# omron-sinicx/neural-astar

Hardware: AMD Instinct MI355X
Metric: map-instances/s (forward A*) 32x32 Moore-8 @batch 4096 (higher is better)
Workload: dtype f32

## Files before the change

### neural-astar_amd/csrc/nastar_forward_compact_body.inc

```
    extern __shared__ __attribute__((aligned(16))) unsigned char smem[];
    if constexpr (kTicket && kRanked) {
        if (ticket_word != nullptr && blockIdx.x == 0 && threadIdx.x == 0)
            __hip_atomic_store(ticket_word, ticket_value, __ATOMIC_RELAXED, __HIP_MEMORY_SCOPE_SYSTEM);
    }
    const int b = kRanked ? ranked_map(levels, a.B) : placed_map(a.order, a.order_bad, a.B);
    if constexpr (kTicket && !kRanked) {
        if (ticket_word != nullptr && blockIdx.x == 0 && threadIdx.x == 0)
            __hip_atomic_store(ticket_word, ticket_value, __ATOMIC_RELAXED, __HIP_MEMORY_SCOPE_SYSTEM);
        asm volatile("s_nop 0\n s_nop 0\n s_nop 0\n s_nop 0\n s_nop 0\n s_nop 0\n s_nop 0\n s_nop 0\n s_nop 0\n s_nop 0\n s_nop 0\n s_nop 0\n s_nop 0\n s_nop 0");
    }
    if ((unsigned)b >= (unsigned)a.B) return;
    const bool lockstep = !kAsm && (a.flags & NASTAR_FLAG_LOCKSTEP);
    if (lockstep && a.marks != nullptr && a.marks[b] == 0) return;
    const int lane = threadIdx.x;
    CompactDims d = a.d;
    if constexpr (LOGH > 0 && LOGW > 0) {
        d.H = 1 << LOGH;
        d.W = 1 << LOGW;
        d.HW = 1 << (LOGH + LOGW);
        d.nchunks = d.HW >> CCL;
        d.HWp = d.HW;
        d.CPL = (d.nchunks + 63) / 64;
        d.NCp = d.CPL * 64;
        d.magicW = (uint32_t)((1ull << 32) >> LOGW) + 1u;
    }
    CompactLds l;
    if constexpr (kAsm) {
        l = carve_compact_asm_lds(smem, d);
        compact_store_guard_rows(l, d, lane);
    } else l = carve_compact_lds(smem, d);
    const size_t off = (size_t)b * (size_t)d.HW;

    int start_idx, goal_idx;
    constexpr int kLoadIter = (kVec4 && LOGH > 0 && LOGW > 0 && LOGH + LOGW >= 8) ? (1 << (LOGH + LOGW - 8)) : 0;
    bool any_signed = true;
    bool all_unit = false;
    compact_load_map<kVec4, kLoadIter>(d, l, a.cost + off, a.start + off, a.goal + off, a.passable + off, lane, start_idx, goal_idx,
                                       kAsm ? &any_signed : nullptr, kAsm ? &all_unit : nullptr);
#ifdef NASTAR_DEV
    const bool raw = kAsm && !any_signed && !(a.flags & NASTAR_FLAG_ASM_V2) && d.gr >= 0.f && d.omg >= 0.f;
#else
    const bool raw = kAsm && !any_signed && d.gr >= 0.f && d.omg >= 0.f;
#endif
    float* hhv = nullptr;
    bool bad_h0 = false;
    if constexpr (kHeur) {
        hhv = reinterpret_cast<float*>(l.pdir + d.HWp);
        bad_h0 = compact_load_heuristic<kVec4>(d, l, hhv, h0 + off, lane);
    }
    const int gi = goal_idx < 0 ? 0 : goal_idx;
    const int goal_r = (int)row_magic((uint32_t)gi, d.magicW, d.W);
    const int goal_c = gi - goal_r * d.W;

    const CompactLane lc = make_compact_lane<kMasked>(d, lane, nmask);
    int status = NASTAR_OK;
    int iters = 0;
    bool solved = false, coupled = false;
    bool goal_hit = false;
    bool stored_h = false;
    const bool probe = lockstep && a.bitmap != nullptr;
    const int budget = (lockstep && a.t_end != nullptr) ? __builtin_amdgcn_readfirstlane(*a.t_end + 1) : a.max_iters;
    uint32_t bits = 0u;
    uint32_t* const bm = probe ? a.bitmap + (size_t)b * (size_t)a.bitmap_words : nullptr;
    if (kHeur && bad_h0) {
        status = NASTAR_ERR_BAD_HEURISTIC;
    } else if (start_idx < 0 || goal_idx < 0) {
        status = NASTAR_ERR_UNSOLVABLE;
    } else {
#ifdef NASTAR_DEV
        const bool asm4 = raw && !(a.flags & NASTAR_FLAG_ASM_V3);
        const bool no_dive = (a.flags & NASTAR_FLAG_NO_DIVE) != 0;
#else
        const bool asm4 = raw;
#endif
        const bool half = asm4 && d.gr == 0.5f && d.omg == 0.5f;
        if constexpr (kMulti) compact_open_sources<kVec4, kFastDiv, kHeur>(d, l, hhv, a.start + off, lane, goal_r, goal_c, rcp_sqrtW);
        else
        if constexpr (kHeur) {
            if (lane == 0) {
                l.gc[start_idx].x = 0.0f;
                l.cmin[start_idx >> CCL] = cmin_entry(compact_key<kFastDiv>(d, 0.0f, hhv[start_idx], rcp_sqrtW), (uint32_t)start_idx);
                l.pdir[start_idx] = (uint8_t)(PARENT_UNSET | P_PASS);
            }
            wave_sync();
        } else
        compact_open_start<kFastDiv>(d, l, lane, start_idx, goal_r, goal_c, rcp_sqrtW, raw, half);
        int s = 0;
        if constexpr (kAsm) {
#ifdef NASTAR_DEV
            stored_h = asm4 && !no_dive && all_unit && a.cost == a.passable;
#else
            stored_h = asm4 && all_unit && a.cost == a.passable;
#endif
            if (stored_h) {
                const bool start_blocked = l.gc[start_idx].y == 0.0f;
                compact_store_heuristic<LOGW>(l, lane, goal_r, goal_c);
                if (start_blocked && lane == 0) l.gc[start_idx].x = -1.0f;
                wave_sync();
            }
            static_assert(LOGW > 0 && LOGW == LOGH && (CPL_T == 1 || CPL_T == 4) && kFastDiv, "asm loop: 16x16, 32x32, 64x64");
            int* const log_row = kLog ? a.sel_log + (size_t)b * (size_t)a.max_iters : nullptr;
            __builtin_amdgcn_s_setprio(3);
            constexpr bool kD = CPL_T == 4;
#ifdef NASTAR_DEV
            if (asm4 && kD && no_dive) {
                if (half) s = search_loop_asm4<LOGW, kLog, false, true, false>(d.gr, d.omg, d.sqrtW, lane, goal_idx, goal_r, goal_c, a.max_iters, iters, rcp_sqrtW, log_row);
                else s = search_loop_asm4<LOGW, kLog, false, false, false>(d.gr, d.omg, d.sqrtW, lane, goal_idx, goal_r, goal_c, a.max_iters, iters, rcp_sqrtW, log_row);
            } else if (raw && !asm4 && kD && no_dive) {
                s = compact_search_loop_asm3<LOGW, kLog, false>(d, lane, goal_idx, goal_r, goal_c, a.max_iters, iters, rcp_sqrtW, log_row);
            } else if (raw && !asm4) {
                s = compact_search_loop_asm3<LOGW, kLog>(d, lane, goal_idx, goal_r, goal_c, a.max_iters, iters, rcp_sqrtW, log_row);
            } else
#endif
            if (stored_h) {
                s = half ? search_loop_asm5<LOGW, kLog, kD, true>(d.gr, d.omg, d.sqrtW, lane, goal_idx, a.max_iters, iters, rcp_sqrtW, log_row)
                         : search_loop_asm5<LOGW, kLog, kD, false>(d.gr, d.omg, d.sqrtW, lane, goal_idx, a.max_iters, iters, rcp_sqrtW, log_row);
            } else if (asm4) {
                s = half ? search_loop_asm4<LOGW, kLog, kD, true, false>(d.gr, d.omg, d.sqrtW, lane, goal_idx, goal_r, goal_c, a.max_iters, iters, rcp_sqrtW, log_row)
                         : search_loop_asm4<LOGW, kLog, kD, false, false>(d.gr, d.omg, d.sqrtW, lane, goal_idx, goal_r, goal_c, a.max_iters, iters, rcp_sqrtW, log_row);
            } else {
                s = compact_search_loop_asm<LOGW, kLog>(d, lane, goal_idx, goal_r, goal_c, a.max_iters, iters, rcp_sqrtW, log_row);
            }
            __builtin_amdgcn_s_setprio(0);
        } else
        while (iters < budget) {
            uint2 mine;
            s = compact_select<CPL_T>(d, l, lane, mine);
            if (s < 0 || (s == goal_idx && !lockstep)) break;
            if constexpr (kLog) {
                if (lane == 0) a.sel_log[(size_t)b * (size_t)a.max_iters + iters] = s;
            }
            if (probe) {
                if (s == goal_idx) bits |= 1u << (iters & 31);
                if ((iters & 31) == 31) {
                    if (lane == 0) bm[iters >> 5] = bits;
                    bits = 0u;
                }
            }
            ++iters;
            goal_hit |= s == goal_idx;
            if constexpr (kHeur) compact_expand<LOGW, kFastDiv, CPL_T, true>(d, l, lc, lane, s, goal_r, goal_c, rcp_sqrtW, mine, s == goal_idx, hhv);
            else
            compact_expand<LOGW, kFastDiv, CPL_T>(d, l, lc, lane, s, goal_r, goal_c, rcp_sqrtW, mine, s == goal_idx);
        }
        if (probe) {
            if (lane == 0) {
                if (iters & 31) bm[iters >> 5] = bits;
                for (int w = (iters + 31) >> 5; w < a.bitmap_words; ++w) bm[w] = 0u;
            }
            return;
        }
        if (lockstep && goal_hit && lane == 0) l.gc[goal_idx].x = NASTAR_NEG_INF;
        if (kAsm ? (s != -2) : (iters < budget)) {
            if (s < 0) {
                status = NASTAR_ERR_UNSOLVABLE;
            } else {
                if constexpr (kLog) {
                    if (lane == 0) a.sel_log[(size_t)b * (size_t)a.max_iters + iters] = s;
                }
                ++iters;
                solved = true;
                if (a.summary != nullptr || a.marks_out != nullptr) {
                    const int nr = goal_r + lc.dr, nc = goal_c + lc.dc;
                    const bool inb = lc.is_nb & ((unsigned)nr < (unsigned)d.H) & ((unsigned)nc < (unsigned)d.W);
                    const int n = inb ? s + lc.off : s;
                    float2 gg = l.gc[s], gn = l.gc[n];
                    if constexpr (kAsm) {
                        if (stored_h) {
                            gn.y = 1.0f;
                            gg.y = 1.0f;
                            if (s == start_idx) gg = make_float2(0.0f, a.cost[off + s]);
                        }
                    }
                    const float g2 = gg.x + gg.y;
                    uint32_t kn, kg;
                    if constexpr (kHeur) {
                        kn = compact_key<kFastDiv>(d, g2, hhv[n], rcp_sqrtW);
                        kg = compact_key<kFastDiv>(d, gg.x, hhv[s], rcp_sqrtW);
                    } else {
                    kn = compact_key<kFastDiv>(d, g2, d.omg * (heuristic0_fast(nr, nc, goal_r, goal_c) + gn.y), rcp_sqrtW);
                    kg = compact_key<kFastDiv>(d, gg.x, d.omg * (heuristic0_fast(goal_r, goal_c, goal_r, goal_c) + gg.y), rcp_sqrtW);
                    }
                    const bool beats = inb & (gn.x > g2) & ((kn < kg) | ((kn == kg) & (n < s)));
                    coupled = __ballot(beats) != 0ull;
                    if (coupled && a.summary != nullptr && lane == 0) a.summary[NASTAR_SUMMARY_COUPLED] = 1;
                    wave_order();
                }
                if (lane == 0) l.gc[s].x = NASTAR_NEG_INF;
            }
        }
    }
    wave_sync();
    compact_store_hist<kVec4>(d, l, lane, a.hist + off);
    if (probe) return;
    if (lane == 0) {
        a.iters[b] = iters;
        a.status[b] = status;
        if (a.marks_out != nullptr) a.marks_out[b] = coupled ? 1 : 0;
        if (status != NASTAR_OK && a.summary) a.summary[status] = 1;
        if (a.order_out) note_completion(a.order_out, a.B, b);
        if (a.done_counter) note_done(a.done_counter, a.summary, a.B, status != NASTAR_OK || coupled);
    }
    if (goal_idx >= 0 && !(kHeur && bad_h0)) compact_backtrack<(LOGW == LOGH ? LOGW : 0)>(d, l, lane, kMulti ? -1 : start_idx, goal_idx, solved ? d.HW : iters - 1);
    compact_store_outputs<kVec4, false>(d, l, lane, a.hist + off, a.paths + off,
                                        a.packed ? a.packed + (size_t)b * (size_t)(d.HW >> 2) : nullptr);
    const RouteOut ro = kernel_route_args<offsetof(FwdCArgs, route)>();
    if (ro.routes != nullptr) {
        const float start_cost = (kAsm && stored_h) ? a.cost[off + start_idx] : 0.f;
        const int n = route_walk(l.pdir, lane, kMulti ? -1 : start_idx, goal_idx, solved ? d.HW : iters - 1, goal_idx >= 0 && !(kHeur && bad_h0),
                                 [&](int c, uint32_t code) { return compact_parent_of(d, c, code); },
                                 [&](int c) { return (kAsm && stored_h) ? (c == start_idx ? start_cost : 1.0f) : l.gc[c].y; }, ro, b);
        route_fill_tail(ro, b, n, lane);
    }
```

### neural-astar_amd/csrc/nastar_search_asm.hip.h

```cpp
#pragma once
#include "nastar_search_compact.hip.h"

namespace nastar {

template <int LOGW>
struct AsmLayout {
    static constexpr int W = 1 << LOGW;
    static constexpr int HW = W * W;
    static constexpr int CPL = (HW / 16 + 63) / 64;
    static constexpr int GC = W * 8;
    static constexpr int CMIN = GC + HW * 8 + W * 8;
    static constexpr int PDIR = CMIN + CPL * 64 * 8;
    static constexpr int BYTES = PDIR + HW;
};
static_assert(AsmLayout<5>::BYTES == (int)compact_asm_lds_bytes(32, 1024, 64) && AsmLayout<5>::BYTES * 16 == 160 * 1024, "16 maps of 32x32 per CU");
static_assert(AsmLayout<6>::BYTES == (int)compact_asm_lds_bytes(64, 4096, 256) && AsmLayout<4>::BYTES == (int)compact_asm_lds_bytes(16, 256, 64), "host and stream agree");

#define NASTAR_ASM_ENTRY \
        "s_cmp_ge_u32 %[it], %[maxit]\n\t" \
        "s_cbranch_scc1 .Lbudget%=\n\t" \
        "v_mov_b32 v48, -1\n\t" \
        "v_mov_b32 v49, -1\n\t"
 \

#define NASTAR_ASM_READ_1 \
        "ds_read_b64 v[20:21], %[l8] offset:%[CMIN]\n\t"
#define NASTAR_ASM_READ_4 \
        "ds_read_b128 v[12:15], %[l8] offset:%[CMIN]\n\t" \
        "ds_read_b128 v[16:19], %[l8] offset:%[CMIN16]\n\t"
#define NASTAR_ASM_LOOPTOP \
        ".Lloop%=:\n\t" \
        "s_waitcnt lgkmcnt(0)\n\t"
#define NASTAR_ASM_LOCALMIN_1
 \

#define NASTAR_ASM_LOCALMIN_4 \
        "v_min_u32 v21, v13, v15\n\t" \
        "v_min3_u32 v21, v21, v17, v19\n\t" \
        "v_mov_b32 v20, v18\n\t" \
        "v_cmp_eq_u32 vcc, v21, v17\n\t" \
        "v_cmp_eq_u32_e64 s[48:49], v21, v15\n\t" \
        "v_cmp_eq_u32_e64 s[50:51], v21, v13\n\t" \
        "v_cndmask_b32 v20, v20, v16, vcc\n\t" \
        "v_cndmask_b32_e64 v20, v20, v14, s[48:49]\n\t" \
        "v_cndmask_b32_e64 v20, v20, v12, s[50:51]\n\t"
#define NASTAR_ASM_SELECT \
  \
        "v_min_u32_dpp v22, v21, v21 quad_perm:[1,0,3,2] row_mask:0xf bank_mask:0xf\n\t" \
        "s_nop 1\n\t" \
        "v_min_u32_dpp v22, v22, v22 quad_perm:[2,3,0,1] row_mask:0xf bank_mask:0xf\n\t" \
        "s_nop 1\n\t" \
        "v_min_u32_dpp v22, v22, v22 row_half_mirror row_mask:0xf bank_mask:0xf\n\t" \
        "s_nop 1\n\t" \
        "v_min_u32_dpp v22, v22, v22 row_mirror row_mask:0xf bank_mask:0xf\n\t" \
        "s_nop 1\n\t" \
        "v_min_u32_dpp v22, v22, v22 row_bcast:15 row_mask:0xa bank_mask:0xf\n\t" \
        "s_nop 1\n\t" \
        "v_min_u32_dpp v22, v22, v22 row_bcast:31 row_mask:0xc bank_mask:0xf\n\t" \
        "s_nop 0\n\t" \
        "v_readlane_b32 s40, v22, 63\n\t"  \
        "s_cmp_eq_u32 s40, -1\n\t" \
        "s_cbranch_scc1 .Lempty%=\n\t"  \
        "v_cmp_eq_u32 vcc, s40, v21\n\t" \
        "s_ff1_i32_b64 s41, vcc\n\t"  \
        "v_readlane_b32 s42, v20, s41\n\t"  \
        "s_cmp_eq_u32 s42, %[goal]\n\t" \
        "s_cbranch_scc1 .Lgoal%=\n\t"
#define NASTAR_ASM_LOG \
        "s_lshl_b32 s53, %[it], 2\n\t"                     \
        "v_mov_b32 v53, s53\n\t"                                                                                           \
        "v_mov_b32 v54, s42\n\t"                                                                                           \
        "s_mov_b64 exec, 1\n\t"                                                                                            \
        "global_store_dword v53, v54, %[logp]\n\t"                                                                         \
        "s_mov_b64 exec, -1\n\t"
#define NASTAR_ASM_EXPAND \
        "s_add_u32 %[it], %[it], 1\n\t" \
  \
        "s_lshr_b32 s43, s42, %[LOGW]\n\t"  \
        "s_and_b32 s44, s42, %[WM1]\n\t"  \
        "s_and_b32 s45, s42, 0xfffffff0\n\t"  \
        "v_add_u32 v23, s43, %[dr]\n\t" \
        "v_add_u32 v24, s44, %[dc]\n\t" \
        "v_max_u32 v23, v23, v24\n\t" \
        "v_cmp_gt_u32 vcc, %[W], v23\n\t"  \
        "v_mov_b32 v24, s42\n\t" \
        "v_mov_b32 v46, s45\n\t" \
        "v_cndmask_b32_e64 v46, v24, v46, %[mchk]\n\t"  \
        "v_add_u32 v46, v46, %[off]\n\t" \
        "s_and_b64 s[54:55], vcc, %[mnb]\n\t"  \
        "v_cndmask_b32 v46, v24, v46, vcc\n\t"  \
        "v_lshlrev_b32 v27, 3, v24\n\t" \
        "v_lshlrev_b32 v26, 3, v46\n\t" \
        "ds_read_b64 v[28:29], v27 offset:%[GC]\n\t"  \
        "ds_read_b64 v[30:31], v26 offset:%[GC]\n\t"  \
  \
        "v_lshrrev_b32 v32, %[LOGW], v46\n\t" \
        "v_and_b32 v33, %[WM1], v46\n\t" \
        "v_subrev_u32 v32, %[gr], v32\n\t" \
        "v_subrev_u32 v33, %[gc], v33\n\t" \
        "v_cvt_f32_i32 v32, v32\n\t" \
        "v_cvt_f32_i32 v33, v33\n\t" \
        "v_mul_f32 v34, v32, v32\n\t" \
        "v_mul_f32 v35, v33, v33\n\t" \
        "v_add_f32 v34, v34, v35\n\t" \
        "v_sqrt_f32 v34, v34\n\t" \
        "v_add_f32_e64 v35, |v32|, |v33|\n\t" \
        "v_min_f32_e64 v32, |v32|, |v33|\n\t" \
        "v_sub_f32 v35, v35, v32\n\t"  \
        "v_mul_f32 v34, 0x3a83126f, v34\n\t"  \
        "v_add_f32 v34, v35, v34\n\t"  \
        "s_lshr_b32 s47, s42, 4\n\t" \
        "s_lshl_b32 s47, s47, 3\n\t"  \
        "s_and_b32 s46, s42, 15\n\t" \
        "s_add_u32 s46, s46, 16\n\t"  \
        "s_waitcnt lgkmcnt(0)\n\t" \
        "v_add_f32 v34, v34, v31\n\t"  \
        "v_mul_f32 v34, %[comg], v34\n\t"  \
        "v_add_f32 v40, v28, v29\n\t"  \
        "v_cndmask_b32_e64 v41, v30, v40, %[mnb]\n\t"  \
        "v_mul_f32 v41, %[cgr], v41\n\t" \
        "v_add_f32 v41, v41, v34\n\t"  \
        "v_mul_f32 v42, %[crcp], v41\n\t"  \
        "v_fma_f32 v43, -v42, %[csq], v41\n\t" \
        "v_fma_f32 v42, v43, %[crcp], v42\n\t" \
        "v_ashrrev_i32 v43, 31, v42\n\t" \
        "v_cmp_eq_u32 vcc, s46, %[lane]\n\t" \
        "v_bitop3_b32 v47, v43, v42, %[msb] bitop3:0x36\n\t"  \
        "v_cndmask_b32_e64 v45, %[vinf], v40, s[54:55]\n\t"  \
        "v_cndmask_b32 v44, %[loc], %[vinf], vcc\n\t"  \
        "v_lshrrev_b32 v50, 4, v46\n\t" \
        "v_lshlrev_b32 v50, 3, v50\n\t"  \
        "v_mov_b32 v52, s47\n\t" \
  \
        "s_mov_b64 exec, 0x100\n\t" \
        "ds_write_b32 v27, %[vminf] offset:%[GC]\n\t" \
        "ds_write_b64 v52, v[48:49] offset:%[CMIN]\n\t" \
        "s_mov_b64 exec, -1\n\t" \
        "v_cmpx_gt_f32 vcc, v30, v44\n\t"  \
        "v_cmpx_ge_f32 vcc, 0x7f7fffff, v30\n\t"  \
        "ds_min_u64 v50, v[46:47] offset:%[CMIN]\n\t" \
        "s_mov_b64 exec, -1\n\t" \
        "v_cmpx_gt_f32 vcc, v30, v45\n\t"  \
        "ds_write_b32 v26, v40 offset:%[GC]\n\t"  \
        "ds_write_b8 v46, %[pcode] offset:%[PDIR]\n\t"  \
        "ds_min_u64 v50, v[46:47] offset:%[CMIN]\n\t"  \
        "s_mov_b64 exec, -1\n\t"
#define NASTAR_ASM_LOOPEND \
        "s_cmp_lt_u32 %[it], %[maxit]\n\t" \
        "s_cbranch_scc1 .Lloop%=\n" \
        ".Lbudget%=:\n\t" \
        "s_waitcnt lgkmcnt(0)\n\t"  \
        "s_mov_b32 %[sel], -2\n\t" \
        "s_branch .Lend%=\n" \
        ".Lempty%=:\n\t" \
        "s_mov_b32 %[sel], -1\n\t" \
        "s_branch .Lend%=\n" \
        ".Lgoal%=:\n\t" \
        "s_mov_b32 %[sel], s42\n" \
        ".Lend%=:\n\t"
#define NASTAR_ASM_OPERANDS \
        : [it] "+s"(it), [sel] "=s"(sel) \
        : [l8] "v"(v_l8), [lane] "v"(lane), [dr] "v"(v_dr), [dc] "v"(v_dc), [off] "v"(v_off), [pcode] "v"(v_pcode), \
          [vinf] "v"(v_inf), [vminf] "v"(v_minf), [loc] "v"(v_loc), [goal] "s"(goal_idx), [gr] "s"(goal_r), [gc] "s"(goal_c), \
          [maxit] "s"(max_iters), [cgr] "s"(d.gr), [comg] "s"(d.omg), [csq] "s"(d.sqrtW), [crcp] "s"(rcp_sqrtW), \
          [mnb] "s"(m_nb), [mchk] "s"(m_chk), [msb] "s"(msb), [logp] "s"(logp), \
          [GC] "i"(L::GC), [CMIN] "i"(L::CMIN), [CMIN16] "i"(L::CMIN + 16), [PDIR] "i"(L::PDIR), [LOGW] "i"(LOGW), [WM1] "i"(L::W - 1), [W] "i"(L::W) \
        : "memory", "vcc", "scc", "v20", "v21", "v22", "v23", "v24", "v26", "v27", "v28", "v29", "v30", "v31", "v32", "v33", \
          "v34", "v35", "v40", "v41", "v42", "v43", "v44", "v45", "v46", "v47", "v48", "v49", "v50", "v52", "s40", "s41", "s42", \
          "s43", "s44", "s45", "s46", "s47", "s50", "s51", "s52", "s54", "s55", "s53", "v53", "v54", "v12", "v13", "v14", "v15", "v16", "v17", "v18", "v19", "s48", "s49"

template <int LOGW, bool kLog>
__device__ __forceinline__ int compact_search_loop_asm(const CompactDims& d, int lane, int goal_idx, int goal_r, int goal_c,
                                                       int max_iters, int& iters, float rcp_sqrtW, int* log_row)
{
    using L = AsmLayout<LOGW>;
    static_assert((L::CPL == 1 || L::CPL == 4) && L::HW >= 256, "1 or 4 chunk minima per lane, chunks inside one map row");
    int dr, dc;
    neighbour_delta(lane & 7, dr, dc);
    const bool is_nb = lane < 8, is_chk = (lane & 48) == 16;
    const int v_dr = is_nb ? dr : 0, v_dc = is_nb ? dc : 0;
    const int v_off = is_nb ? dr * L::W + dc : (is_chk ? (lane & 15) : 0);
    const uint32_t v_pcode = P_PASS | (uint32_t)(lane & 7);
    const uint32_t v_l8 = (uint32_t)lane * 8u * L::CPL;
    const float v_inf = NASTAR_POS_INF, v_minf = NASTAR_NEG_INF;
    const float v_loc = is_chk ? NASTAR_NEG_INF : NASTAR_POS_INF;
    const unsigned long long m_nb = 0xFFull, m_chk = 0xFFFF0000ull;
    const uint32_t msb = 0x80000000u;
    int it = __builtin_amdgcn_readfirstlane(iters);
    goal_idx = __builtin_amdgcn_readfirstlane(goal_idx);
    goal_r = __builtin_amdgcn_readfirstlane(goal_r);
    goal_c = __builtin_amdgcn_readfirstlane(goal_c);
    max_iters = __builtin_amdgcn_readfirstlane(max_iters);
    int sel;
    unsigned long long logp = reinterpret_cast<unsigned long long>(log_row);
#define NASTAR_ASM_BODY(N, LOGPART) \
    NASTAR_ASM_ENTRY NASTAR_ASM_READ_##N NASTAR_ASM_LOOPTOP NASTAR_ASM_LOCALMIN_##N NASTAR_ASM_SELECT LOGPART NASTAR_ASM_EXPAND \
        NASTAR_ASM_READ_##N NASTAR_ASM_LOOPEND
    if constexpr (L::CPL == 1) {
        if constexpr (kLog) asm volatile(NASTAR_ASM_BODY(1, NASTAR_ASM_LOG) NASTAR_ASM_OPERANDS);
        else asm volatile(NASTAR_ASM_BODY(1, ) NASTAR_ASM_OPERANDS);
    } else {
        if constexpr (kLog) asm volatile(NASTAR_ASM_BODY(4, NASTAR_ASM_LOG) NASTAR_ASM_OPERANDS);
        else asm volatile(NASTAR_ASM_BODY(4, ) NASTAR_ASM_OPERANDS);
    }
#undef NASTAR_ASM_BODY
    iters = it;
    return sel;
}

}
```

### neural-astar_amd/csrc/nastar_search_asm3.hip.h

```cpp
#pragma once
#include "nastar_search_asm.hip.h"

namespace nastar {

#define NASTAR_ASM3_SELECT \
  \
        "v_min_u32_dpp v22, v21, v21 quad_perm:[1,0,3,2] row_mask:0xf bank_mask:0xf\n\t" \
        "v_min_u32_dpp v23, v21, v21 quad_perm:[2,3,0,1] row_mask:0xf bank_mask:0xf\n\t" \
        "v_min_u32_dpp v22, v21, v22 quad_perm:[3,2,1,0] row_mask:0xf bank_mask:0xf\n\t" \
        "v_min_u32 v22, v22, v23\n\t" \
        "s_add_u32 %[it], %[it], 1\n\t" \
        "s_nop 0\n\t" \
        "v_min_u32_dpp v22, v22, v22 row_half_mirror row_mask:0xf bank_mask:0xf\n\t" \
        "s_nop 1\n\t" \
        "v_min_u32_dpp v22, v22, v22 row_mirror row_mask:0xf bank_mask:0xf\n\t" \
        "s_nop 1\n\t" \
        "v_min_u32_dpp v22, v22, v22 row_bcast:15 row_mask:0xa bank_mask:0xf\n\t" \
        "s_nop 1\n\t" \
        "v_min_u32_dpp v22, v22, v22 row_bcast:31 row_mask:0xc bank_mask:0xf\n\t" \
        "s_nop 0\n\t" \
        "v_readlane_b32 s40, v22, 63\n\t"  \
        "s_cmp_eq_u32 s40, -1\n\t" \
        "s_cbranch_scc1 .Lempty%=\n\t"  \
        "v_cmp_eq_u32 vcc, s40, v21\n\t" \
        "s_ff1_i32_b64 s41, vcc\n\t"  \
        "v_readlane_b32 s42, v20, s41\n\t"  \
        "s_cmp_eq_u32 s42, %[goal]\n\t" \
        "s_cbranch_scc1 .Lgoal%=\n\t"
#define NASTAR_ASM3_LOG \
        "s_lshl_b32 s53, %[it], 2\n\t"                     \
        "s_sub_u32 s53, s53, 4\n\t"                                                                                        \
        "v_mov_b32 v53, s53\n\t"                                                                                           \
        "v_mov_b32 v54, s42\n\t"                                                                                           \
        "s_mov_b64 exec, 1\n\t"                                                                                            \
        "global_store_dword v53, v54, %[logp]\n\t"                                                                         \
        "s_mov_b64 exec, -1\n\t"
#define NASTAR_ASM3_LOOPEND \
        "s_cmp_lt_u32 %[it], %[maxit]\n\t" \
        "s_cbranch_scc1 .Lloop%=\n" \
        ".Lbudget%=:\n\t" \
        "s_waitcnt lgkmcnt(0)\n\t"  \
        "s_mov_b32 %[sel], -2\n\t" \
        "s_branch .Lend%=\n" \
        ".Lempty%=:\n\t" \
        "s_sub_u32 %[it], %[it], 1\n\t"  \
        "s_mov_b32 %[sel], -1\n\t" \
        "s_branch .Lend%=\n" \
        ".Lgoal%=:\n\t" \
        "s_sub_u32 %[it], %[it], 1\n\t"  \
        "s_mov_b32 %[sel], s42\n" \
        ".Lend%=:\n\t"

#define NASTAR_ASM3_X_PREFIX \
        "s_lshr_b32 s43, s42, %[LOGW]\n\t"  \
        "s_and_b32 s44, s42, %[WM1]\n\t"  \
        "v_add_u32 v32, s43, %[dr]\n\t"  \
        "v_and_b32 v33, s44, %[cmask]\n\t"  \
        "v_add_u32 v33, v33, %[dcc]\n\t"  \
        "v_mov_b32 v24, s42\n\t" \
        "v_max_u32 v23, v32, v33\n\t" \
        "v_lshl_add_u32 v46, v32, %[LOGW], v33\n\t"  \
        "v_cmp_gt_u32 vcc, %[W], v23\n\t"  \
        "v_lshlrev_b32 v27, 3, v24\n\t" \
        "ds_read_b64 v[28:29], v27 offset:%[GC]\n\t"  \
        "s_and_b64 s[54:55], vcc, %[mnb]\n\t"  \
        "v_cndmask_b32 v46, v24, v46, vcc\n\t"  \
        "v_lshlrev_b32 v26, 3, v46\n\t" \
        "v_lshrrev_b32 v50, 4, v46\n\t" \
        "v_lshlrev_b32 v50, 3, v50\n\t"
#define NASTAR_ASM3_X_CLOSE \
  \
        "s_mov_b64 exec, 0x100\n\t" \
        "ds_write_b32 v27, %[vminf] offset:%[GC]\n\t" \
        "ds_write_b64 v50, v[48:49] offset:%[CMIN]\n\t" \
        "s_mov_b64 exec, -1\n\t"
#define NASTAR_ASM3_X_READCELL \
        "ds_read_b64 v[30:31], v26 offset:%[GC]\n\t"
#define NASTAR_ASM3_X_HEUR \
  \
        "v_sad_u32 v35, v32, %[gr], 0\n\t"  \
        "v_sad_u32 v36, v33, %[gc], 0\n\t"  \
        "v_max_u32 v37, v35, v36\n\t"  \
        "v_mul_u32_u24 v34, v35, v35\n\t" \
        "v_mad_u32_u24 v34, v36, v36, v34\n\t" \
        "v_cvt_f32_u32 v34, v34\n\t" \
        "v_sqrt_f32 v34, v34\n\t" \
        "v_cvt_f32_u32 v37, v37\n\t"  \
        "v_mul_f32 v34, 0x3a83126f, v34\n\t"  \
        "v_add_f32 v34, v37, v34\n\t"
#define NASTAR_ASM3_X_WAIT \
        "s_waitcnt lgkmcnt(0)\n\t"
#define NASTAR_ASM3_X_KEY \
        "v_add_f32 v34, v34, v31\n\t"  \
        "v_add_f32 v40, v28, v29\n\t"  \
        "v_mul_f32 v34, %[comg], v34\n\t"  \
        "v_cndmask_b32_e64 v41, v30, v40, %[mnb]\n\t"  \
        "v_mul_f32 v41, %[cgr], v41\n\t" \
        "v_add_f32 v41, v41, v34\n\t"  \
        "v_mul_f32 v42, %[crcp], v41\n\t"  \
        "v_fma_f32 v43, -v42, %[csq], v41\n\t" \
        "v_fma_f32 v47, v43, %[crcp], v42\n\t"
#define NASTAR_ASM3_X_RELAX(SET55) \
  \
        "v_cmp_class_f32_e64 s[58:59], v30, %[cls]\n\t"  \
        "s_mov_b64 exec, s[54:55]\n\t" \
        "v_cmpx_gt_f32 vcc, v30, v40\n\t"  \
        SET55 \
        "ds_write_b32 v26, v40 offset:%[GC]\n\t"  \
        "ds_write_b8 v46, %[pcode] offset:%[PDIR]\n\t"  \
        "s_or_b64 exec, exec, s[58:59]\n\t" \
        "ds_min_u64 v50, v[46:47] offset:%[CMIN]\n\t"  \
        "s_mov_b64 exec, -1\n\t"
#define NASTAR_ASM3_EXPAND_(INIT55, SET55) \
    NASTAR_ASM3_X_PREFIX NASTAR_ASM3_X_CLOSE NASTAR_ASM3_X_READCELL INIT55 NASTAR_ASM3_X_HEUR NASTAR_ASM3_X_WAIT NASTAR_ASM3_X_KEY \
        NASTAR_ASM3_X_RELAX(SET55)
#define NASTAR_ASM3_EXPAND NASTAR_ASM3_EXPAND_(, )
#define NASTAR_ASM3_EXPAND_DIVE NASTAR_ASM3_EXPAND_(, "v_cmp_lt_u32_e64 s[60:61], v47, s40\n\t")

#define NASTAR_ASM3_DIVE_TEST \
        "s_cmp_ge_u32 %[it], %[maxit]\n\t" \
        "s_cbranch_scc1 .Lbudget%=\n\t" \
        "s_cmp_lg_u64 s[60:61], 0\n\t"  \
        "s_cbranch_scc1 .Ldive%=\n\t"
#define NASTAR_ASM3_DIVE_LOOKUP \
        ".Ldive%=:\n\t" \
        "v_cndmask_b32_e64 v55, v48, v47, s[60:61]\n\t"  \
        "s_nop 1\n\t" \
        "v_min_u32_dpp v56, v55, v55 quad_perm:[1,0,3,2] row_mask:0xf bank_mask:0xf\n\t" \
        "v_min_u32_dpp v57, v55, v55 quad_perm:[2,3,0,1] row_mask:0xf bank_mask:0xf\n\t" \
        "v_min_u32_dpp v56, v55, v56 quad_perm:[3,2,1,0] row_mask:0xf bank_mask:0xf\n\t" \
        "v_min_u32 v56, v56, v57\n\t" \
        "s_add_u32 %[it], %[it], 1\n\t" \
        "s_nop 0\n\t" \
        "v_min_u32_dpp v56, v56, v56 row_half_mirror row_mask:0xf bank_mask:0xf\n\t" \
        "s_nop 0\n\t" \
        "v_readfirstlane_b32 s56, v56\n\t"  \
        "s_mov_b32 s40, s56\n\t"  \
        "s_nop 0\n\t" \
        "v_cmp_eq_u32 vcc, s56, v55\n\t" \
        "s_ff1_i32_b64 s41, vcc\n\t"  \
        "v_readlane_b32 s42, v46, s41\n\t"  \
        "s_cmp_eq_u32 s42, %[goal]\n\t" \
        "s_cbranch_scc1 .Lgoal%=\n" \
        ".Lselected%=:\n\t"
#define NASTAR_ASM3_EXITS \
        ".Lbudget%=:\n\t" \
        "s_waitcnt lgkmcnt(0)\n\t"  \
        "s_mov_b32 %[sel], -2\n\t" \
        "s_branch .Lend%=\n" \
        ".Lempty%=:\n\t" \
        "s_sub_u32 %[it], %[it], 1\n\t" \
        "s_mov_b32 %[sel], -1\n\t" \
        "s_branch .Lend%=\n" \
        ".Lgoal%=:\n\t" \
        "s_sub_u32 %[it], %[it], 1\n\t" \
        "s_mov_b32 %[sel], s42\n" \
        ".Lend%=:\n\t"


#define NASTAR_ASM3_OPERANDS \
        : [it] "+s"(it), [sel] "=s"(sel) \
        : [l8] "v"(v_l8), [dr] "v"(v_dr), [cmask] "v"(v_cmask), [dcc] "v"(v_dcc), [pcode] "v"(v_pcode), [cls] "v"(v_cls), \
          [vminf] "v"(v_minf), [goal] "s"(goal_idx), [gr] "s"(goal_r), [gc] "s"(goal_c), \
          [maxit] "s"(max_iters), [cgr] "s"(d.gr), [comg] "s"(d.omg), [csq] "s"(d.sqrtW), [crcp] "s"(rcp_sqrtW), \
          [mnb] "s"(m_nb), [logp] "s"(logp), \
          [GC] "i"(L::GC), [CMIN] "i"(L::CMIN), [CMIN16] "i"(L::CMIN + 16), [PDIR] "i"(L::PDIR), [LOGW] "i"(LOGW), [WM1] "i"(L::W - 1), [W] "i"(L::W) \
        : "memory", "vcc", "scc", "v20", "v21", "v22", "v23", "v24", "v26", "v27", "v28", "v29", "v30", "v31", "v32", "v33", \
          "v34", "v35", "v36", "v37", "v40", "v41", "v42", "v43", "v46", "v47", "v48", "v49", "v50", "s40", "s41", "s42", \
          "s43", "s44", "s54", "s55", "s53", "v53", "v54", "v12", "v13", "v14", "v15", "v16", "v17", "v18", "v19", "s48", "s49", \
          "s50", "s51", "v55", "v56", "v57", "s56", "s58", "s59", "s60", "s61"

template <int LOGW, bool kLog, bool kDive = true>
__device__ __forceinline__ int compact_search_loop_asm3(const CompactDims& d, int lane, int goal_idx, int goal_r, int goal_c,
                                                        int max_iters, int& iters, float rcp_sqrtW, int* log_row)
{
    using L = AsmLayout<LOGW>;
    static_assert((L::CPL == 1 || L::CPL == 4) && L::HW >= 256, "1 or 4 chunk minima per lane, chunks inside one map row");
    int dr, dc;
    neighbour_delta(lane & 7, dr, dc);
    const bool is_nb = lane < 8, is_chk = (lane & 48) == 16;
    const int v_dr = is_nb ? dr : 0;
    const int v_dcc = is_nb ? dc : (is_chk ? (lane & 15) : 0);
    const uint32_t v_cmask = is_chk ? 0xFFFFFFF0u : 0xFFFFFFFFu;
    const uint32_t v_cls = is_chk ? 0x1F8u : 0u;
    const uint32_t v_pcode = P_PASS | (uint32_t)(lane & 7);
    const uint32_t v_l8 = (uint32_t)lane * 8u * L::CPL;
    const float v_minf = NASTAR_NEG_INF;
    const unsigned long long m_nb = 0xFFull;
    int it = __builtin_amdgcn_readfirstlane(iters);
    goal_idx = __builtin_amdgcn_readfirstlane(goal_idx);
    goal_r = __builtin_amdgcn_readfirstlane(goal_r);
    goal_c = __builtin_amdgcn_readfirstlane(goal_c);
    max_iters = __builtin_amdgcn_readfirstlane(max_iters);
    int sel;
    unsigned long long logp = reinterpret_cast<unsigned long long>(log_row);
#define NASTAR_ASM3_BODY(N, LOGPART) \
    NASTAR_ASM_ENTRY NASTAR_ASM_READ_##N NASTAR_ASM_LOOPTOP NASTAR_ASM_LOCALMIN_##N NASTAR_ASM3_SELECT LOGPART NASTAR_ASM3_EXPAND \
        NASTAR_ASM_READ_##N NASTAR_ASM3_LOOPEND
#define NASTAR_ASM3_BODY_DIVE(N, LOGPART) \
    NASTAR_ASM_ENTRY NASTAR_ASM_READ_##N "s_branch .Lsel%=\n" NASTAR_ASM3_DIVE_LOOKUP LOGPART NASTAR_ASM3_EXPAND_DIVE NASTAR_ASM_READ_##N \
        NASTAR_ASM3_DIVE_TEST ".Lsel%=:\n\t" "s_waitcnt lgkmcnt(0)\n\t" NASTAR_ASM_LOCALMIN_##N NASTAR_ASM3_SELECT \
        "s_branch .Lselected%=\n" NASTAR_ASM3_EXITS
    if constexpr (L::CPL == 1) {
        if constexpr (kLog) asm volatile(NASTAR_ASM3_BODY(1, NASTAR_ASM3_LOG) NASTAR_ASM3_OPERANDS);
        else asm volatile(NASTAR_ASM3_BODY(1, ) NASTAR_ASM3_OPERANDS);
    } else if constexpr (kDive) {
        if constexpr (kLog) asm volatile(NASTAR_ASM3_BODY_DIVE(4, NASTAR_ASM3_LOG) NASTAR_ASM3_OPERANDS);
        else asm volatile(NASTAR_ASM3_BODY_DIVE(4, ) NASTAR_ASM3_OPERANDS);
    } else {
        if constexpr (kLog) asm volatile(NASTAR_ASM3_BODY(4, NASTAR_ASM3_LOG) NASTAR_ASM3_OPERANDS);
        else asm volatile(NASTAR_ASM3_BODY(4, ) NASTAR_ASM3_OPERANDS);
    }
#undef NASTAR_ASM3_BODY_DIVE
#undef NASTAR_ASM3_BODY
    iters = it;
    return sel;
}

}
```

### neural-astar_amd/csrc/nastar_search_asm4.hip.h

```cpp
#pragma once
#include "nastar_search_asm3.hip.h"

namespace nastar {

template <int LOGW>
struct AsmLayoutUnit {
    static constexpr int W = 1 << LOGW;
    static constexpr int HW = W * W;
    static constexpr int CPL = (HW / 16 + 63) / 64;
    static constexpr int GC = 0;
    static constexpr int CMIN = HW * 4;
    static constexpr int PDIR = CMIN + CPL * 64 * 8;
    static constexpr int BYTES = PDIR + HW;
};

#define NASTAR_ASM4_ENTRY \
        "s_cmp_ge_u32 %[it], %[maxit]\n\t" \
        "s_cbranch_scc1 .Lbudget%=\n\t" \
        "v_mov_b32 v48, %[goal]\n\t"  \
        "v_mov_b32 v49, -1\n\t"

#define NASTAR_ASM4_SELECT \
        "v_min_u32_dpp v22, v21, v21 quad_perm:[1,0,3,2] row_mask:0xf bank_mask:0xf\n\t" \
        "v_min_u32_dpp v23, v21, v21 quad_perm:[2,3,0,1] row_mask:0xf bank_mask:0xf\n\t" \
        "v_min_u32_dpp v22, v21, v22 quad_perm:[3,2,1,0] row_mask:0xf bank_mask:0xf\n\t" \
        "v_min_u32 v22, v22, v23\n\t" \
        "s_nop 1\n\t" \
        "v_min_u32_dpp v22, v22, v22 row_half_mirror row_mask:0xf bank_mask:0xf\n\t" \
        "s_nop 1\n\t" \
        "v_min_u32_dpp v22, v22, v22 row_mirror row_mask:0xf bank_mask:0xf\n\t" \
        "s_nop 1\n\t" \
        "v_min_u32_dpp v22, v22, v22 row_bcast:15 row_mask:0xa bank_mask:0xf\n\t" \
        "s_nop 1\n\t" \
        "v_min_u32_dpp v22, v22, v22 row_bcast:31 row_mask:0xc bank_mask:0xf\n\t" \
        "s_nop 0\n\t" \
        "v_readlane_b32 s40, v22, 63\n\t"  \
        "s_add_u32 %[it], %[it], 1\n\t"  \
        "s_nop 0\n\t" \
        "v_cmp_eq_u32 vcc, s40, v21\n\t" \
        "s_ff1_i32_b64 s41, vcc\n\t" \
        "v_readlane_b32 s42, v20, s41\n\t" \
        "s_cmp_eq_u32 s42, %[goal]\n\t" \
        "s_cbranch_scc1 .Lgoal%=\n\t"

#define NASTAR_ASM4_X_PREFIX(SH, RDS) \
        "s_lshr_b32 s43, s42, %[LOGW]\n\t"  \
        "s_and_b32 s44, s42, %[WM1]\n\t"  \
        "v_add_u32 v32, s43, %[dr]\n\t"  \
        "v_and_b32 v33, s44, %[cmask]\n\t" \
        "v_add_u32 v33, v33, %[dcc]\n\t"  \
        "v_mov_b32 v24, s42\n\t" \
        "v_max_u32 v23, v32, v33\n\t" \
        "v_lshl_add_u32 v46, v32, %[LOGW], v33\n\t"  \
        "v_cmp_gt_u32 vcc, %[W], v23\n\t"  \
        "v_lshlrev_b32 v27, " SH ", v24\n\t" \
        RDS  \
        "v_lshlrev_b32 v26, " SH ", v46\n\t" \
        "s_and_b64 s[54:55], vcc, %[mnb]\n\t"  \
        "v_lshrrev_b32 v50, 4, v46\n\t" \
        "v_lshlrev_b32 v50, 3, v50\n\t"

#define NASTAR_ASM4_X_KEY(ADDH, ADDG, MULH, MULG) \
        ADDH  \
        ADDG  \
        MULH  \
        "v_cndmask_b32_e64 v41, v30, v40, %[mnb]\n\t"  \
        MULG  \
        "v_add_f32 v41, v41, v34\n\t"  \
        "v_mul_f32 v42, %[crcp], v41\n\t"  \
        "v_fma_f32 v43, -v42, %[csq], v41\n\t" \
        "v_fma_f32 v47, v43, %[crcp], v42\n\t"

#define NASTAR_ASM4_DIVE_LOOKUP \
        ".Ldive%=:\n\t" \
        "v_cndmask_b32_e64 v55, v49, v47, s[60:61]\n\t" \
        "s_nop 1\n\t" \
        "v_min_u32_dpp v56, v55, v55 quad_perm:[1,0,3,2] row_mask:0xf bank_mask:0xf\n\t" \
        "v_min_u32_dpp v57, v55, v55 quad_perm:[2,3,0,1] row_mask:0xf bank_mask:0xf\n\t" \
        "v_min_u32_dpp v56, v55, v56 quad_perm:[3,2,1,0] row_mask:0xf bank_mask:0xf\n\t" \
        "v_min_u32 v56, v56, v57\n\t" \
        "s_add_u32 %[it], %[it], 1\n\t" \
        "s_nop 0\n\t" \
        "v_min_u32_dpp v56, v56, v56 row_half_mirror row_mask:0xf bank_mask:0xf\n\t" \
        "s_nop 0\n\t" \
        "v_readfirstlane_b32 s56, v56\n\t" \
        "s_mov_b32 s40, s56\n\t" \
        "s_nop 0\n\t" \
        "v_cmp_eq_u32 vcc, s56, v55\n\t" \
        "s_ff1_i32_b64 s41, vcc\n\t" \
        "v_readlane_b32 s42, v46, s41\n\t" \
        "s_cmp_eq_u32 s42, %[goal]\n\t" \
        "s_cbranch_scc1 .Lgoal%=\n" \
        ".Lselected%=:\n\t"

#define NASTAR_ASM4_EXITS \
        ".Lbudget%=:\n\t" \
        "s_waitcnt lgkmcnt(0)\n\t"  \
        "s_mov_b32 %[sel], -2\n\t" \
        "s_branch .Lend%=\n" \
        ".Lgoal%=:\n\t" \
        "s_sub_u32 %[it], %[it], 1\n\t"  \
        "s_mov_b32 %[sel], s42\n\t" \
        "s_mov_b32 %[mkey], s40\n" \
        ".Lend%=:\n\t"
#define NASTAR_ASM4_LOOPEND \
        "s_cmp_lt_u32 %[it], %[maxit]\n\t" \
        "s_cbranch_scc1 .Lloop%=\n" \
        NASTAR_ASM4_EXITS

#define NASTAR_ASM4_OPERANDS \
        : [it] "+s"(it), [sel] "=s"(sel), [mkey] "=s"(mkey) \
        : [l8] "v"(v_l8), [dr] "v"(v_dr), [cmask] "v"(v_cmask), [dcc] "v"(v_dcc), [pcode] "v"(v_pcode), [cls] "v"(v_cls), \
          [vminf] "v"(v_minf), [goal] "s"(goal_idx), [gr] "s"(goal_r), [gc] "s"(goal_c), \
          [maxit] "s"(max_iters), [cgr] "s"(cgr), [comg] "s"(comg), [csq] "s"(csq), [crcp] "s"(rcp_sqrtW), \
          [mnb] "s"(m_nb), [logp] "s"(logp), \
          [GC] "i"(GC), [CMIN] "i"(CMIN), [CMIN16] "i"(CMIN + 16), [PDIR] "i"(PDIR), [LOGW] "i"(LOGW), [WM1] "i"((1 << LOGW) - 1), [W] "i"(1 << LOGW) \
        : "memory", "vcc", "scc", "v20", "v21", "v22", "v23", "v24", "v26", "v27", "v28", "v29", "v30", "v31", "v32", "v33", \
          "v34", "v35", "v36", "v37", "v40", "v41", "v42", "v43", "v46", "v47", "v48", "v49", "v50", "s40", "s41", "s42", \
          "s43", "s44", "s54", "s55", "s53", "v53", "v54", "v12", "v13", "v14", "v15", "v16", "v17", "v18", "v19", "s48", "s49", \
          "s50", "s51", "v55", "v56", "v57", "s56", "s58", "s59", "s60", "s61"

template <int LOGW, bool kLog, bool kDive, bool kHalf, bool kUnit>
__device__ __forceinline__ int search_loop_asm4(float cgr, float comg, float csq, int lane, int goal_idx, int goal_r, int goal_c,
                                                int max_iters, int& iters, float rcp_sqrtW, int* log_row)
{
    using LG = AsmLayout<LOGW>;
    using LU = AsmLayoutUnit<LOGW>;
    constexpr int CPL = LG::CPL;
    constexpr int GC = kUnit ? LU::GC : LG::GC;
    constexpr int CMIN = kUnit ? LU::CMIN : LG::CMIN;
    constexpr int PDIR = kUnit ? LU::PDIR : LG::PDIR;
    static_assert((CPL == 1 || CPL == 4) && LG::HW >= 256, "1 or 4 chunk minima per lane, chunks inside one map row");
    int dr, dc;
    neighbour_delta(lane & 7, dr, dc);
    const bool is_nb = lane < 8, is_chk = (lane & 48) == 16;
    const int v_dr = is_nb ? dr : 0;
    const int v_dcc = is_nb ? dc : (is_chk ? (lane & 15) : 0);
    const uint32_t v_cmask = is_chk ? 0xFFFFFFF0u : 0xFFFFFFFFu;
    const uint32_t v_cls = is_chk ? 0x1F8u : 0u;
    const uint32_t v_pcode = P_PASS | (uint32_t)(lane & 7);
    const uint32_t v_l8 = (uint32_t)lane * 8u * CPL;
    const float v_minf = NASTAR_NEG_INF;
    const unsigned long long m_nb = 0xFFull;
    int it = __builtin_amdgcn_readfirstlane(iters);
    goal_idx = __builtin_amdgcn_readfirstlane(goal_idx);
    goal_r = __builtin_amdgcn_readfirstlane(goal_r);
    goal_c = __builtin_amdgcn_readfirstlane(goal_c);
    max_iters = __builtin_amdgcn_readfirstlane(max_iters);
    int sel;
    uint32_t mkey = 0;
    unsigned long long logp = reinterpret_cast<unsigned long long>(log_row);
#define NASTAR_A4_SH_G "3"
#define NASTAR_A4_SH_U "2"
#define NASTAR_A4_RDS_G "ds_read_b64 v[28:29], v27 offset:%[GC]\n\t"
#define NASTAR_A4_RDS_U "ds_read_b32 v28, v27 offset:%[GC]\n\t"
#define NASTAR_A4_RDC_G "ds_read_b64 v[30:31], v26 offset:%[GC]\n\t"
#define NASTAR_A4_RDC_U "ds_read_b32 v30, v26 offset:%[GC]\n\t"
#define NASTAR_A4_ADDH_G "v_add_f32 v34, v34, v31\n\t"
#define NASTAR_A4_ADDH_U "v_add_f32 v34, 1.0, v34\n\t"
#define NASTAR_A4_ADDG_G "v_add_f32 v40, v28, v29\n\t"
#define NASTAR_A4_ADDG_U "v_add_f32 v40, 1.0, v28\n\t"
#define NASTAR_A4_MULH "v_mul_f32 v34, %[comg], v34\n\t"
#define NASTAR_A4_MULG "v_mul_f32 v41, %[cgr], v41\n\t"
#define NASTAR_A4_EXPAND(L, MH, MG, SET55) \
    NASTAR_ASM4_X_PREFIX(NASTAR_A4_SH_##L, NASTAR_A4_RDS_##L) NASTAR_ASM3_X_CLOSE NASTAR_A4_RDC_##L NASTAR_ASM3_X_HEUR NASTAR_ASM3_X_WAIT \
        NASTAR_ASM4_X_KEY(NASTAR_A4_ADDH_##L, NASTAR_A4_ADDG_##L, MH, MG) NASTAR_ASM3_X_RELAX(SET55)
#define NASTAR_A4_BODY(N, L, MH, MG, LOGPART) \
    NASTAR_ASM4_ENTRY NASTAR_ASM_READ_##N NASTAR_ASM_LOOPTOP NASTAR_ASM_LOCALMIN_##N NASTAR_ASM4_SELECT LOGPART NASTAR_A4_EXPAND(L, MH, MG, ) \
        NASTAR_ASM_READ_##N NASTAR_ASM4_LOOPEND
#define NASTAR_A4_BODY_DIVE(N, L, MH, MG, LOGPART) \
    NASTAR_ASM4_ENTRY NASTAR_ASM_READ_##N "s_branch .Lsel%=\n" NASTAR_ASM4_DIVE_LOOKUP LOGPART \
        NASTAR_A4_EXPAND(L, MH, MG, "v_cmp_lt_u32_e64 s[60:61], v47, s40\n\t") NASTAR_ASM_READ_##N NASTAR_ASM3_DIVE_TEST ".Lsel%=:\n\t" \
        "s_waitcnt lgkmcnt(0)\n\t" NASTAR_ASM_LOCALMIN_##N NASTAR_ASM4_SELECT "s_branch .Lselected%=\n" NASTAR_ASM4_EXITS
#define NASTAR_A4_RUN2(BODY, N, L, MH, MG) \
    do { \
        if constexpr (kLog) asm volatile(BODY(N, L, MH, MG, NASTAR_ASM3_LOG) NASTAR_ASM4_OPERANDS); \
        else asm volatile(BODY(N, L, MH, MG, ) NASTAR_ASM4_OPERANDS); \
    } while (0)
#define NASTAR_A4_RUN(BODY, N) \
    do { \
        if constexpr (kUnit && kHalf) NASTAR_A4_RUN2(BODY, N, U, , ); \
        else if constexpr (kUnit) NASTAR_A4_RUN2(BODY, N, U, NASTAR_A4_MULH, NASTAR_A4_MULG); \
        else if constexpr (kHalf) NASTAR_A4_RUN2(BODY, N, G, , ); \
        else NASTAR_A4_RUN2(BODY, N, G, NASTAR_A4_MULH, NASTAR_A4_MULG); \
    } while (0)
    if constexpr (CPL == 1 && kDive) NASTAR_A4_RUN(NASTAR_A4_BODY_DIVE, 1);
    else if constexpr (CPL == 1) NASTAR_A4_RUN(NASTAR_A4_BODY, 1);
    else if constexpr (kDive) NASTAR_A4_RUN(NASTAR_A4_BODY_DIVE, 4);
    else NASTAR_A4_RUN(NASTAR_A4_BODY, 4);
#undef NASTAR_A4_RUN
#undef NASTAR_A4_RUN2
#undef NASTAR_A4_BODY_DIVE
#undef NASTAR_A4_BODY
#undef NASTAR_A4_EXPAND
    iters = it;
    return (sel >= 0 && mkey == 0xFFFFFFFFu) ? -1 : sel;
}


}
```

### neural-astar_amd/csrc/nastar_search_asm5.hip.h

```cpp
#pragma once
#include "nastar_search_asm4.hip.h"

namespace nastar {

#define NASTAR_ASM5_ENTRY \
        "s_mov_b32 s55, 0\n\t"
#define NASTAR_ASM5_X_PREFIX \
        "v_and_b32 v46, s42, %[cmask]\n\t"  \
        "v_lshlrev_b32_e64 v27, 3, s42\n\t" \
        "v_add_u32 v46, v46, %[delta]\n\t"  \
        "ds_read_b32 v28, v27 offset:%[GC]\n\t"  \
        "v_lshlrev_b32 v26, 3, v46\n\t"
#define NASTAR_ASM5_X_CLOSE \
  \
        "s_mov_b64 exec, 0x100\n\t" \
        "ds_write_b32 v27, %[vminf] offset:%[GC]\n\t" \
        "s_mov_b64 exec, -1\n\t"
#define NASTAR_ASM5_X_READCELL \
        "ds_read_b64 v[30:31], v26 offset:%[GC]\n\t"
#define NASTAR_ASM5_X_SHADOW \
  \
        "v_readlane_b32 s54, %[colmask], s42\n\t" \
        "v_lshrrev_b32 v50, 4, v46\n\t" \
        "v_lshlrev_b32 v50, 3, v50\n\t"  \
        "s_mov_b64 exec, 0x100\n\t" \
        "ds_write_b64 v50, v[48:49] offset:%[CMIN]\n\t" \
        "s_mov_b64 exec, -1\n\t"
#define NASTAR_ASM5_X_WAIT \
        "s_waitcnt lgkmcnt(1)\n\t"
#define NASTAR_ASM5_X_KEY(MULH, MULG) \
        "v_add_f32 v40, 1.0, v28\n\t"  \
        MULH  \
        "v_cndmask_b32_e64 v41, v30, v40, %[mnb]\n\t"  \
        MULG  \
        "v_add_f32 v41, v41, v31\n\t"  \
        "v_mul_f32 v42, %[crcp], v41\n\t"  \
        "v_fma_f32 v43, -v42, %[csq], v41\n\t" \
        "v_fma_f32 v47, v43, %[crcp], v42\n\t"
#define NASTAR_ASM5_MULH "v_mul_f32 v31, %[comg], v31\n\t"
#define NASTAR_ASM5_MULG "v_mul_f32 v41, %[cgr], v41\n\t"

#define NASTAR_ASM5_OPERANDS \
        : [it] "+s"(it), [sel] "=s"(sel), [mkey] "=s"(mkey) \
        : [l8] "v"(v_l8), [cmask] "v"(v_cmask), [colmask] "v"(v_colmask), [delta] "v"(v_delta), [pcode] "v"(v_pcode), \
          [cls] "v"(v_cls), [vminf] "v"(v_minf), [goal] "s"(goal_idx), \
          [maxit] "s"(max_iters), [cgr] "s"(cgr), [comg] "s"(comg), [csq] "s"(csq), [crcp] "s"(rcp_sqrtW), \
          [mnb] "s"(m_nb), [logp] "s"(logp), \
          [GC] "i"(GC), [CMIN] "i"(CMIN), [CMIN16] "i"(CMIN + 16), [PDIR] "i"(PDIR) \
        : "memory", "vcc", "scc", "v20", "v21", "v22", "v23", "v26", "v27", "v28", "v30", "v31", \
          "v40", "v41", "v42", "v43", "v46", "v47", "v48", "v49", "v50", "s40", "s41", "s42", \
          "s54", "s55", "s53", "v53", "v54", "v12", "v13", "v14", "v15", "v16", "v17", "v18", "v19", "s48", "s49", \
          "s50", "s51", "v55", "v56", "v57", "s56", "s58", "s59", "s60", "s61"

template <int LOGW, bool kLog, bool kDive, bool kHalf>
__device__ __forceinline__ int search_loop_asm5(float cgr, float comg, float csq, int lane, int goal_idx, int max_iters, int& iters,
                                                float rcp_sqrtW, int* log_row)
{
    using LG = AsmLayout<LOGW>;
    constexpr int CPL = LG::CPL;
    constexpr int GC = LG::GC;
    constexpr int CMIN = LG::CMIN;
    constexpr int PDIR = LG::PDIR;
    static_assert((CPL == 1 || CPL == 4) && LG::HW >= 256, "1 or 4 chunk minima per lane, chunks inside one map row");
    int dr, dc;
    neighbour_delta(lane & 7, dr, dc);
    const bool is_nb = lane < 8, is_chk = (lane & 48) == 16;
    const int v_delta = is_nb ? dr * (1 << LOGW) + dc : (is_chk ? (lane & 15) : 0);
    const uint32_t v_cmask = is_chk ? 0xFFFFFFF0u : 0xFFFFFFFFu;
    const uint32_t v_cls = is_chk ? 0x1F8u : 0u;
    const uint32_t v_pcode = P_PASS | (uint32_t)(lane & 7);
    const uint32_t v_l8 = (uint32_t)lane * 8u * CPL;
    const float v_minf = NASTAR_NEG_INF;
    const unsigned long long m_nb = 0xFFull;
    const int col = lane & ((1 << LOGW) - 1);
    const uint32_t v_colmask = 0xFFu & ~(col == 0 ? 0x29u : 0u) & ~(col == (1 << LOGW) - 1 ? 0x94u : 0u);
    int it = __builtin_amdgcn_readfirstlane(iters);
    goal_idx = __builtin_amdgcn_readfirstlane(goal_idx);
    max_iters = __builtin_amdgcn_readfirstlane(max_iters);
    int sel;
    uint32_t mkey = 0;
    unsigned long long logp = reinterpret_cast<unsigned long long>(log_row);
#define NASTAR_A5_EXPAND(MH, MG, SET55) \
    NASTAR_ASM5_X_PREFIX NASTAR_ASM5_X_CLOSE NASTAR_ASM5_X_READCELL NASTAR_ASM5_X_SHADOW NASTAR_ASM5_X_WAIT NASTAR_ASM5_X_KEY(MH, MG) \
        NASTAR_ASM3_X_RELAX(SET55)
#define NASTAR_A5_BODY(N, MH, MG, LOGPART) \
    NASTAR_ASM5_ENTRY NASTAR_ASM4_ENTRY NASTAR_ASM_READ_##N NASTAR_ASM_LOOPTOP NASTAR_ASM_LOCALMIN_##N NASTAR_ASM4_SELECT LOGPART NASTAR_A5_EXPAND(MH, MG, ) \
        NASTAR_ASM_READ_##N NASTAR_ASM4_LOOPEND
#define NASTAR_A5_BODY_DIVE(N, MH, MG, LOGPART) \
    NASTAR_ASM5_ENTRY NASTAR_ASM4_ENTRY NASTAR_ASM_READ_##N "s_branch .Lsel%=\n" NASTAR_ASM4_DIVE_LOOKUP LOGPART \
        NASTAR_A5_EXPAND(MH, MG, "v_cmp_lt_u32_e64 s[60:61], v47, s40\n\t") NASTAR_ASM_READ_##N NASTAR_ASM3_DIVE_TEST ".Lsel%=:\n\t" \
        "s_waitcnt lgkmcnt(0)\n\t" NASTAR_ASM_LOCALMIN_##N NASTAR_ASM4_SELECT "s_branch .Lselected%=\n" NASTAR_ASM4_EXITS
#define NASTAR_A5_RUN2(BODY, N, MH, MG) \
    do { \
        if constexpr (kLog) asm volatile(BODY(N, MH, MG, NASTAR_ASM3_LOG) NASTAR_ASM5_OPERANDS); \
        else asm volatile(BODY(N, MH, MG, ) NASTAR_ASM5_OPERANDS); \
    } while (0)
#define NASTAR_A5_RUN(BODY, N) \
    do { \
        if constexpr (kHalf) NASTAR_A5_RUN2(BODY, N, , ); \
        else NASTAR_A5_RUN2(BODY, N, NASTAR_ASM5_MULH, NASTAR_ASM5_MULG); \
    } while (0)
    if constexpr (CPL == 1 && kDive) NASTAR_A5_RUN(NASTAR_A5_BODY_DIVE, 1);
    else if constexpr (CPL == 1) NASTAR_A5_RUN(NASTAR_A5_BODY, 1);
    else if constexpr (kDive) NASTAR_A5_RUN(NASTAR_A5_BODY_DIVE, 4);
    else NASTAR_A5_RUN(NASTAR_A5_BODY, 4);
#undef NASTAR_A5_RUN
#undef NASTAR_A5_RUN2
#undef NASTAR_A5_BODY_DIVE
#undef NASTAR_A5_BODY
#undef NASTAR_A5_EXPAND
    iters = it;
    return (sel >= 0 && mkey == 0xFFFFFFFFu) ? -1 : sel;
}

template <int LOGW>
__device__ __forceinline__ void compact_store_heuristic(const CompactLds& l, int lane, int goal_r, int goal_c)
{
    constexpr int W = 1 << LOGW, HW = W * W;
    static_assert(W <= 64 && HW % 64 == 0, "a lane's cells share one column");
    const int c = lane & (W - 1);
    const int dcol = c > goal_c ? c - goal_c : goal_c - c;
    const uint32_t dc2 = (uint32_t)(dcol * dcol);
#pragma unroll 4
    for (int k = 0; k < HW / 64; ++k) {
        const int i = lane + 64 * k;
        const int r = i >> LOGW;
        const int drow = r > goal_r ? r - goal_r : goal_r - r;
        const uint32_t cheb = (uint32_t)(drow > dcol ? drow : dcol);
        const float euc = __builtin_amdgcn_sqrtf((float)((uint32_t)(drow * drow) + dc2));
        const float h0 = (float)cheb + 0.001f * euc;
        l.gc[i].y = h0 + 1.0f;
    }
}

}
```

### neural-astar_amd/csrc/nastar_search_compact.hip.h

```cpp
#pragma once
#include "nastar_search.hip.h"

namespace nastar {

constexpr int CCL = 4;
constexpr int CCSZ = 1 << CCL;

struct CompactDims {
    int H, W, HW;
    int nchunks;
    int HWp;
    int CPL;
    int NCp;
    uint32_t magicW;
    float gr, omg, sqrtW;
};

struct CompactLds {
    float2* gc;
    unsigned long long* cmin;
    uint8_t* pdir;
    uint32_t* dump;
};

__host__ __device__ inline size_t compact_lds_bytes(int HWp, int NCp) { return (size_t)HWp * 9 + (size_t)NCp * 8 + 256; }

__host__ __device__ constexpr size_t compact_asm_lds_bytes(int W, int HWp, int NCp) { return (size_t)HWp * 9 + (size_t)NCp * 8 + (size_t)W * 16; }
__host__ __device__ inline bool compact_asm_shape(int H, int W) { return H == W && (W == 16 || W == 32 || W == 64); }

__host__ __device__ inline size_t compact_launch_lds_bytes(int H, int W, int HWp, int NCp, bool asm_stream)
{
    return (asm_stream && compact_asm_shape(H, W)) ? compact_asm_lds_bytes(W, HWp, NCp) : compact_lds_bytes(HWp, NCp);
}

__host__ __device__ inline size_t compact_heur_lds_bytes(int HWp, int NCp) { return compact_lds_bytes(HWp, NCp) + (size_t)HWp * 4; }

__device__ __forceinline__ CompactLds carve_compact_lds(unsigned char* smem, const CompactDims& d)
{
    CompactLds l;
    l.gc = reinterpret_cast<float2*>(smem);
    l.cmin = reinterpret_cast<unsigned long long*>(l.gc + d.HWp);
    l.dump = reinterpret_cast<uint32_t*>(l.cmin + d.NCp);
    l.pdir = reinterpret_cast<uint8_t*>(l.dump + 64);
    return l;
}

__device__ __forceinline__ CompactLds carve_compact_asm_lds(unsigned char* smem, const CompactDims& d)
{
    CompactLds l;
    l.gc = reinterpret_cast<float2*>(smem) + d.W;
    l.cmin = reinterpret_cast<unsigned long long*>(l.gc + d.HW + d.W);
    l.pdir = reinterpret_cast<uint8_t*>(l.cmin + d.NCp);
    l.dump = nullptr;
    return l;
}

__device__ __forceinline__ void compact_store_guard_rows(const CompactLds& l, const CompactDims& d, int lane)
{
    for (int i = lane; i < 2 * d.W; i += 64) l.gc[i < d.W ? i - d.W : d.HW + i - d.W] = make_float2(NASTAR_NEG_INF, 0.f);
}

__device__ __forceinline__ unsigned long long cmin_entry(uint32_t key, uint32_t idx)
{
    return ((unsigned long long)key << 32) | (unsigned long long)idx;
}

template <bool kFastDiv>
__device__ __forceinline__ uint32_t compact_key(const CompactDims& d, float G, float hh, float rcp_sqrtW)
{
    const float f = d.gr * G + hh;
    float q;
    if constexpr (kFastDiv) {
        const float q0 = f * rcp_sqrtW;
        const float rem = __builtin_fmaf(-q0, d.sqrtW, f);
        q = __builtin_fmaf(rem, rcp_sqrtW, q0);
    } else {
        q = f / d.sqrtW;
    }
    return f32_to_ord(q);
}

__device__ __forceinline__ float heuristic0_fast(int r, int c, int goal_r, int goal_c)
{
    const float a = (float)(r - goal_r);
    const float b = (float)(c - goal_c);
    const float dr = fabsf(a), dc = fabsf(b);
    const float cheb = (dr + dc) - fminf(dr, dc);
    const float euc = sqrt_rn_int(a * a + b * b);
    return cheb + 0.001f * euc;
}

template <bool kVec4, int ITER = 0>
__device__ __forceinline__ void compact_load_map(const CompactDims& d, const CompactLds& l, const float* __restrict__ cost,
                                                 const float* __restrict__ start, const float* __restrict__ goal,
                                                 const float* __restrict__ passable, int lane, int& start_idx, int& goal_idx,
                                                 bool* any_signed = nullptr, bool* all_unit = nullptr)
{
    int sidx = -1, gidx = -1;
    bool sgn = false, nun = false;
    if constexpr (kVec4) {
        const float4* s4 = reinterpret_cast<const float4*>(start);
        const float4* g4 = reinterpret_cast<const float4*>(goal);
        const float4* c4 = reinterpret_cast<const float4*>(cost);
        const float4* p4 = reinterpret_cast<const float4*>(passable);
        auto place = [&](int q, const float4& sv, const float4& gv, const float4& cv, const float4& pv) {
            const int i = q << 2;
            if (sv.x != 0.f) sidx = i;
            if (sv.y != 0.f) sidx = i + 1;
            if (sv.z != 0.f) sidx = i + 2;
            if (sv.w != 0.f) sidx = i + 3;
            if (gv.x != 0.f) gidx = i;
            if (gv.y != 0.f) gidx = i + 1;
            if (gv.z != 0.f) gidx = i + 2;
            if (gv.w != 0.f) gidx = i + 3;
            sgn |= !(cv.x >= 0.f) | !(cv.y >= 0.f) | !(cv.z >= 0.f) | !(cv.w >= 0.f);
            nun |= ((cv.x != 0.f) & (cv.x != 1.f)) | ((cv.y != 0.f) & (cv.y != 1.f)) | ((cv.z != 0.f) & (cv.z != 1.f)) | ((cv.w != 0.f) & (cv.w != 1.f));
            float4 lo, hi;
            lo.x = pv.x != 0.f ? NASTAR_POS_INF : NASTAR_NEG_INF;
            lo.y = cv.x;
            lo.z = pv.y != 0.f ? NASTAR_POS_INF : NASTAR_NEG_INF;
            lo.w = cv.y;
            hi.x = pv.z != 0.f ? NASTAR_POS_INF : NASTAR_NEG_INF;
            hi.y = cv.z;
            hi.z = pv.w != 0.f ? NASTAR_POS_INF : NASTAR_NEG_INF;
            hi.w = cv.w;
            *reinterpret_cast<float4*>(l.gc + i) = lo;
            *reinterpret_cast<float4*>(l.gc + i + 2) = hi;
            const uint32_t m = (PARENT_UNSET | (pv.x != 0.f ? P_PASS : 0u)) | ((PARENT_UNSET | (pv.y != 0.f ? P_PASS : 0u)) << 8) |
                               ((PARENT_UNSET | (pv.z != 0.f ? P_PASS : 0u)) << 16) |
                               ((PARENT_UNSET | (pv.w != 0.f ? P_PASS : 0u)) << 24);
            *reinterpret_cast<uint32_t*>(l.pdir + i) = m;
        };
        if constexpr (ITER > 0) {
            constexpr int G = ITER < 4 ? ITER : 4;
            static_assert(ITER % G == 0, "groups of up to 4 iterations");
            const bool same_cp = passable == cost;
            for (int base = 0; base < ITER; base += G) {
                float4 sv[G], gv[G], cv[G], pv[G];
#pragma unroll
                for (int k = 0; k < G; ++k) {
                    const int q = lane + (base + k) * 64;
                    sv[k] = s4[q];
                    gv[k] = g4[q];
                    cv[k] = c4[q];
                }
                if (same_cp) {
#pragma unroll
                    for (int k = 0; k < G; ++k) pv[k] = cv[k];
                } else {
#pragma unroll
                    for (int k = 0; k < G; ++k) pv[k] = p4[lane + (base + k) * 64];
                }
#pragma unroll
                for (int k = 0; k < G; ++k) place(lane + (base + k) * 64, sv[k], gv[k], cv[k], pv[k]);
            }
        } else {
            const int n4 = d.HW >> 2;
            for (int q = lane; q < n4; q += 64) place(q, s4[q], g4[q], c4[q], p4[q]);
        }
    } else {
        for (int i = lane; i < d.HW; i += 64) {
            if (start[i] != 0.f) sidx = i;
            if (goal[i] != 0.f) gidx = i;
            const float pv = passable[i];
            sgn |= !(cost[i] >= 0.f);
            nun |= (cost[i] != 0.f) & (cost[i] != 1.f);
            l.gc[i] = make_float2(pv != 0.f ? NASTAR_POS_INF : NASTAR_NEG_INF, cost[i]);
            l.pdir[i] = (uint8_t)(PARENT_UNSET | (pv != 0.f ? P_PASS : 0u));
        }
    }
    for (int i = d.HW + lane; i < d.HWp; i += 64) l.gc[i] = make_float2(NASTAR_NEG_INF, 0.f);
    start_idx = wave_max_i32(sidx);
    goal_idx = wave_max_i32(gidx);
    const unsigned long long idle = cmin_entry(0xFFFFFFFFu, (uint32_t)(goal_idx < 0 ? 0 : goal_idx));
    for (int c = lane; c < d.NCp; c += 64) l.cmin[c] = idle;
    if (any_signed != nullptr) *any_signed = __ballot(sgn) != 0ull;
    if (all_unit != nullptr) *all_unit = __ballot(nun) == 0ull;
    wave_sync();
}

template <bool kVec4>
__device__ __forceinline__ bool compact_load_heuristic(const CompactDims& d, const CompactLds& l, float* hhv, const float* __restrict__ h0, int lane)
{
    bool bad = false;
    if constexpr (kVec4) {
        const float4* h4 = reinterpret_cast<const float4*>(h0);
        const int n4 = d.HW >> 2;
        for (int q = lane; q < n4; q += 64) {
            const float4 hv = h4[q];
            const float4 lo = *reinterpret_cast<const float4*>(l.gc + (q << 2));
            const float4 hi = *reinterpret_cast<const float4*>(l.gc + (q << 2) + 2);
            bad = bad || !(fabsf(hv.x) < NASTAR_POS_INF) || !(fabsf(hv.y) < NASTAR_POS_INF) || !(fabsf(hv.z) < NASTAR_POS_INF) || !(fabsf(hv.w) < NASTAR_POS_INF);
            float4 o;
            o.x = d.omg * (hv.x + lo.y);
            o.y = d.omg * (hv.y + lo.w);
            o.z = d.omg * (hv.z + hi.y);
            o.w = d.omg * (hv.w + hi.w);
            *reinterpret_cast<float4*>(hhv + (q << 2)) = o;
        }
    } else {
        for (int i = lane; i < d.HW; i += 64) {
            const float hv = h0[i];
            bad |= !(fabsf(hv) < NASTAR_POS_INF);
            hhv[i] = d.omg * (hv + l.gc[i].y);
        }
    }
    for (int i = d.HW + lane; i < d.HWp; i += 64) hhv[i] = 0.f;
    const bool any_bad = __ballot(bad) != 0ull;
    wave_sync();
    return any_bad;
}

template <bool kFastDiv>
__device__ __forceinline__ void compact_open_start(const CompactDims& d, const CompactLds& l, int lane, int sidx, int goal_r,
                                                   int goal_c, float rcp_sqrtW, bool raw_key = false, bool half_key = false)
{
    if (lane == 0) {
        const int r = (int)row_magic((uint32_t)sidx, d.magicW, d.W);
        const int c = sidx - r * d.W;
        const float hh = (half_key ? 1.0f : d.omg) * (heuristic0_fast(r, c, goal_r, goal_c) + l.gc[sidx].y);
        uint32_t k0 = compact_key<kFastDiv>(d, 0.0f, hh, rcp_sqrtW);
        if (raw_key) k0 = __float_as_uint(ord_to_f32(k0));
        l.gc[sidx].x = 0.0f;
        l.cmin[sidx >> CCL] = cmin_entry(k0, (uint32_t)sidx);
        l.pdir[sidx] = (uint8_t)(PARENT_UNSET | P_PASS);
    }
    wave_sync();
}

template <bool kVec4, bool kFastDiv, bool kHeur>
__device__ __forceinline__ void compact_open_sources(const CompactDims& d, const CompactLds& l, const float* hhv, const float* __restrict__ start,
                                                     int lane, int goal_r, int goal_c, float rcp_sqrtW)
{
    auto open = [&](int i) {
        float hh;
        if constexpr (kHeur) {
            hh = hhv[i];
        } else {
            const int r = (int)row_magic((uint32_t)i, d.magicW, d.W);
            const int c = i - r * d.W;
            hh = d.omg * (heuristic0_fast(r, c, goal_r, goal_c) + l.gc[i].y);
        }
        const uint32_t k0 = compact_key<kFastDiv>(d, 0.0f, hh, rcp_sqrtW);
        l.gc[i].x = 0.0f;
        l.pdir[i] = (uint8_t)(PARENT_UNSET | P_PASS);
        atomicMin(&l.cmin[i >> CCL], cmin_entry(k0, (uint32_t)i));
    };
    if constexpr (kVec4) {
        const float4* s4 = reinterpret_cast<const float4*>(start);
        const int n4 = d.HW >> 2;
        for (int q = lane; q < n4; q += 64) {
            const float4 sv = s4[q];
            if (sv.x != 0.f) open(q << 2);
            if (sv.y != 0.f) open((q << 2) + 1);
            if (sv.z != 0.f) open((q << 2) + 2);
            if (sv.w != 0.f) open((q << 2) + 3);
        }
    } else {
        for (int i = lane; i < d.HW; i += 64)
            if (start[i] != 0.f) open(i);
    }
    wave_sync();
}

template <int CPL_T>
__device__ __forceinline__ int compact_select(const CompactDims& d, const CompactLds& l, int lane, uint2& mine)
{
    uint2 best;
    if constexpr (CPL_T == 1) {
        const unsigned long long e = l.cmin[lane];
        best.x = (uint32_t)e;
        best.y = (uint32_t)(e >> 32);
    } else {
        const int cpl = CPL_T > 0 ? CPL_T : d.CPL;
        const uint2* p = reinterpret_cast<const uint2*>(l.cmin) + lane * cpl;
        best = p[0];
        if constexpr (CPL_T > 0) {
#pragma unroll
            for (int c = 1; c < CPL_T; ++c) {
                const uint2 e = p[c];
                if (e.y < best.y) best = e;
            }
        } else {
            for (int c = 1; c < cpl; ++c) {
                const uint2 e = p[c];
                if (e.y < best.y) best = e;
            }
        }
    }
    mine = best;
    const uint32_t M = wave_min_scalar_u32(best.y);
    const int L = __builtin_ctzll(__ballot(best.y == M));
    const int s = __builtin_amdgcn_readlane((int)best.x, L);
    return M == KEY_INF ? -1 : s;
}

struct CompactLane {
    int dr, dc, off;
    bool is_nb;
    bool is_chk;
    uint32_t pcode;
};

template <bool kMasked = false>
__device__ __forceinline__ CompactLane make_compact_lane(const CompactDims& d, int lane, uint32_t nmask = 0u)
{
    CompactLane lc;
    neighbour_delta(lane & 7, lc.dr, lc.dc);
    lc.is_nb = kMasked ? neighbour_enabled(lane, nmask) : lane < 8;
    lc.is_chk = (lane & 48) == 16;
    lc.off = lc.dr * d.W + lc.dc;
    lc.pcode = P_PASS | (uint32_t)(lane & 7);
    return lc;
}

template <int LOGW, bool kFastDiv, int CPL_T, bool kHeur = false>
__device__ __forceinline__ void compact_expand(const CompactDims& d, const CompactLds& l, const CompactLane& lc, int lane, int s,
                                               int goal_r, int goal_c, float rcp_sqrtW, const uint2 mine, const bool keep_open = false,
                                               const float* hhv = nullptr)
{
    int r, c;
    if constexpr (LOGW) {
        r = s >> LOGW;
        c = s & ((1 << LOGW) - 1);
    } else {
        r = (int)row_magic((uint32_t)s, d.magicW, d.W);
        c = s - r * d.W;
    }
    const int cbase = s & ~(CCSZ - 1);
    const int nr = r + lc.dr, nc = c + lc.dc;
    const bool inb = lc.is_nb & ((unsigned)nr < (unsigned)d.H) & ((unsigned)nc < (unsigned)d.W);
    const int il = inb ? s + lc.off : (lc.is_chk ? cbase + (lane & (CCSZ - 1)) : s);
    const float2 gs = l.gc[s];
    const float2 gl = l.gc[il];
    float hh;
    if constexpr (kHeur) {
        hh = hhv[il];
    } else {
    int rl, cl;
    if constexpr (LOGW) {
        rl = il >> LOGW;
        cl = il & ((1 << LOGW) - 1);
    } else {
        rl = (int)row_magic((uint32_t)il, d.magicW, d.W);
        cl = il - rl * d.W;
    }
    const float h0 = heuristic0_fast(rl, cl, goal_r, goal_c);
    hh = d.omg * (h0 + gl.y);
    }
    const float g2 = gs.x + gs.y;
    const bool upd = inb & (gl.x > g2);
    const uint32_t k = compact_key<kFastDiv>(d, lc.is_nb ? g2 : gl.x, hh, rcp_sqrtW);
    const bool open_l = lc.is_chk & (fabsf(gl.x) < NASTAR_POS_INF) & ((il != s) | keep_open);
    const uint32_t kk = open_l ? k : KEY_INF;
    const uint32_t mc = row_min16_u32(kk);
    const unsigned long long firstm = __ballot(lc.is_chk & (kk == mc));
    const uint32_t Mc = (uint32_t)__builtin_amdgcn_readlane((int)mc, 16);
    const uint32_t ci = (uint32_t)(cbase + __builtin_ctzll(firstm) - 16);
    uint32_t* const dmp = l.dump + lane;
    float* const g_dst = upd ? &l.gc[il].x : ((lane == 8 && !keep_open) ? &l.gc[s].x : reinterpret_cast<float*>(dmp));
    uint8_t* const p_dst = upd ? &l.pdir[il] : reinterpret_cast<uint8_t*>(dmp);
    *g_dst = upd ? g2 : NASTAR_NEG_INF;
    *p_dst = (uint8_t)lc.pcode;
    if constexpr (CPL_T == 1) {
        const bool owner = lane == (s >> CCL);
        uint2 e;
        e.x = owner ? ci : mine.x;
        e.y = owner ? Mc : mine.y;
        reinterpret_cast<uint2*>(l.cmin)[lane] = e;
    } else {
        if (lane == 16) l.cmin[s >> CCL] = cmin_entry(Mc, ci);
    }
    atomicMin(upd ? &l.cmin[il >> CCL] : &l.cmin[lane], upd ? cmin_entry(k, (uint32_t)il) : ~0ull);
    wave_order();
}

__device__ __forceinline__ int compact_parent_of(const CompactDims& d, int n, uint32_t code)
{
    int dr, dc;
    neighbour_delta((int)code, dr, dc);
    return n - (dr * d.W + dc);
}

template <int LOGW = 0>
__device__ __forceinline__ void compact_backtrack(const CompactDims& d, const CompactLds& l, int lane, int start_idx, int goal_idx,
                                                  int cap)
{
    if (lane == 0) {
        auto parent_of = [&](int n, uint32_t code) -> int {
            if constexpr (LOGW > 0 && LOGW <= 6) {
                constexpr int W = 1 << LOGW;
                constexpr unsigned long long LUT =
                    ((unsigned long long)(uint8_t)(int8_t)(-W - 1)) | ((unsigned long long)(uint8_t)(int8_t)(-W) << 8) |
                    ((unsigned long long)(uint8_t)(int8_t)(-W + 1) << 16) | ((unsigned long long)(uint8_t)(int8_t)(-1) << 24) |
                    ((unsigned long long)(uint8_t)(int8_t)(1) << 32) | ((unsigned long long)(uint8_t)(int8_t)(W - 1) << 40) |
                    ((unsigned long long)(uint8_t)(int8_t)(W) << 48) | ((unsigned long long)(uint8_t)(int8_t)(W + 1) << 56);
                return n - (int)(int8_t)(LUT >> (code * 8u));
            } else {
                return compact_parent_of(d, n, code);
            }
        };
        uint32_t m = l.pdir[goal_idx];
        l.pdir[goal_idx] = (uint8_t)(m | P_PATH);
        uint32_t code = m & P_DIRMASK;
        if (code != PARENT_UNSET) {
            int loc = parent_of(goal_idx, code);
            for (int k = 0; k < cap; ++k) {
                uint32_t ml = l.pdir[loc];
                l.pdir[loc] = (uint8_t)(ml | P_PATH);
                if (loc == start_idx) break;
                uint32_t cd = ml & P_DIRMASK;
                if (cd == PARENT_UNSET) break;
                loc = parent_of(loc, cd);
            }
        }
    }
    wave_sync();
}

template <bool kVec4>
__device__ __forceinline__ void compact_store_hist(const CompactDims& d, const CompactLds& l, int lane, float* __restrict__ hist)
{
    if constexpr (kVec4) {
        const int n4 = d.HW >> 2;
        float4* h4 = reinterpret_cast<float4*>(hist);
        for (int q = lane; q < n4; q += 64) {
            const uint32_t m = *reinterpret_cast<const uint32_t*>(l.pdir + (q << 2));
            const float4 lo = *reinterpret_cast<const float4*>(l.gc + (q << 2));
            const float4 hi = *reinterpret_cast<const float4*>(l.gc + (q << 2) + 2);
            float4 v;
            v.x = ((m & P_PASS) && lo.x == NASTAR_NEG_INF) ? 1.0f : 0.0f;
            v.y = ((m & (P_PASS << 8)) && lo.z == NASTAR_NEG_INF) ? 1.0f : 0.0f;
            v.z = ((m & (P_PASS << 16)) && hi.x == NASTAR_NEG_INF) ? 1.0f : 0.0f;
            v.w = ((m & (P_PASS << 24)) && hi.z == NASTAR_NEG_INF) ? 1.0f : 0.0f;
            h4[q] = v;
        }
    } else {
        for (int i = lane; i < d.HW; i += 64) hist[i] = ((l.pdir[i] & P_PASS) && l.gc[i].x == NASTAR_NEG_INF) ? 1.0f : 0.0f;
    }
}

template <bool kVec4, bool kHist = true>
__device__ __forceinline__ void compact_store_outputs(const CompactDims& d, const CompactLds& l, int lane, float* __restrict__ hist,
                                                      long long* __restrict__ paths, uint8_t* __restrict__ packed = nullptr)
{
    if constexpr (kVec4) {
        const int n4 = d.HW >> 2;
        float4* h4 = reinterpret_cast<float4*>(hist);
        if (kHist || packed != nullptr)
        for (int q = lane; q < n4; q += 64) {
            const uint32_t m = *reinterpret_cast<const uint32_t*>(l.pdir + (q << 2));
            const float4 lo = *reinterpret_cast<const float4*>(l.gc + (q << 2));
            const float4 hi = *reinterpret_cast<const float4*>(l.gc + (q << 2) + 2);
            const bool c0 = (m & P_PASS) && lo.x == NASTAR_NEG_INF;
            const bool c1 = (m & (P_PASS << 8)) && lo.z == NASTAR_NEG_INF;
            const bool c2 = (m & (P_PASS << 16)) && hi.x == NASTAR_NEG_INF;
            const bool c3 = (m & (P_PASS << 24)) && hi.z == NASTAR_NEG_INF;
            float4 v;
            v.x = c0 ? 1.0f : 0.0f;
            v.y = c1 ? 1.0f : 0.0f;
            v.z = c2 ? 1.0f : 0.0f;
            v.w = c3 ? 1.0f : 0.0f;
            if (kHist) h4[q] = v;
            if (packed != nullptr) {
                const uint32_t nh = (c0 ? 8u : 0u) | (c1 ? 4u : 0u) | (c2 ? 2u : 0u) | (c3 ? 1u : 0u);
                const uint32_t np = ((m & P_PATH) ? 8u : 0u) | ((m & (P_PATH << 8)) ? 4u : 0u) |
                                    ((m & (P_PATH << 16)) ? 2u : 0u) | ((m & (P_PATH << 24)) ? 1u : 0u);
                const uint32_t both = nh | (np << 8);
                const uint32_t other = dpp_mov<DPP_QUAD_XOR1>(both);
                if ((lane & 1) == 0) {
                    const int nb = d.HW >> 3;
                    packed[q >> 1] = (uint8_t)((nh << 4) | (other & 0xFu));
                    packed[nb + (q >> 1)] = (uint8_t)((np << 4) | ((other >> 8) & 0xFu));
                }
            }
        }
        const int n2 = d.HW >> 1;
        longlong2* p2 = reinterpret_cast<longlong2*>(paths);
        for (int q = lane; q < n2; q += 64) {
            const uint32_t m = *reinterpret_cast<const uint16_t*>(l.pdir + (q << 1));
            longlong2 v;
            v.x = (m & P_PATH) ? 1 : 0;
            v.y = (m & (P_PATH << 8)) ? 1 : 0;
            p2[q] = v;
        }
    } else {
        for (int i = lane; i < d.HW; i += 64) {
            const uint32_t m = l.pdir[i];
            if (kHist) hist[i] = ((m & P_PASS) && l.gc[i].x == NASTAR_NEG_INF) ? 1.0f : 0.0f;
            paths[i] = (m & P_PATH) ? 1 : 0;
        }
    }
}

}
```

Baseline: 37.66 million.

## Use 32-cell chunks for 32x32 asm A* open-list minima

For 32x32 maps the asm search kernels now group cells into chunks of 32 (one full map row) instead of 16, halving the number of chunk-minimum entries to 32. The wave-wide minimum reduction then ends after the row_mirror step with two readlanes and a scalar min, dropping the two row_bcast DPP steps and their nops from every iteration. The chunk-rescan lanes are remapped to the upper 32 lanes so a whole chunk is rescanned in one pass. In exchange, each chunk rescan covers twice as many cells, and every shift, mask and lane constant must stay consistent across the asm variants.

```diff
diff --git a/neural-astar_amd/csrc/nastar_forward_compact_body.inc b/neural-astar_amd/csrc/nastar_forward_compact_body.inc
--- a/neural-astar_amd/csrc/nastar_forward_compact_body.inc
+++ b/neural-astar_amd/csrc/nastar_forward_compact_body.inc
@@ -14,11 +14,12 @@
     if (lockstep && a.marks != nullptr && a.marks[b] == 0) return;
     const int lane = threadIdx.x;
     CompactDims d = a.d;
+    constexpr int kCcl = kAsm ? compact_asm_ccl(LOGW) : CCL;
     if constexpr (LOGH > 0 && LOGW > 0) {
         d.H = 1 << LOGH;
         d.W = 1 << LOGW;
         d.HW = 1 << (LOGH + LOGW);
-        d.nchunks = d.HW >> CCL;
+        d.nchunks = d.HW >> kCcl;
         d.HWp = d.HW;
         d.CPL = (d.nchunks + 63) / 64;
         d.NCp = d.CPL * 64;
@@ -84,7 +85,7 @@
             }
             wave_sync();
         } else
-        compact_open_start<kFastDiv>(d, l, lane, start_idx, goal_r, goal_c, rcp_sqrtW, raw, half);
+        compact_open_start<kFastDiv>(d, l, lane, start_idx, goal_r, goal_c, rcp_sqrtW, raw, half, kCcl);
         int s = 0;
         if constexpr (kAsm) {
 #ifdef NASTAR_DEV
diff --git a/neural-astar_amd/csrc/nastar_search_asm.hip.h b/neural-astar_amd/csrc/nastar_search_asm.hip.h
--- a/neural-astar_amd/csrc/nastar_search_asm.hip.h
+++ b/neural-astar_amd/csrc/nastar_search_asm.hip.h
@@ -7,7 +7,9 @@
 struct AsmLayout {
     static constexpr int W = 1 << LOGW;
     static constexpr int HW = W * W;
-    static constexpr int CPL = (HW / 16 + 63) / 64;
+    static constexpr int CCL = compact_asm_ccl(LOGW);
+    static constexpr int CPL = ((HW >> CCL) + 63) / 64;
+    static constexpr int ROWS = CPL > 1 ? 4 : ((HW >> CCL) + 15) / 16;
     static constexpr int GC = W * 8;
     static constexpr int CMIN = GC + HW * 8 + W * 8;
     static constexpr int PDIR = CMIN + CPL * 64 * 8;
@@ -44,21 +46,33 @@
         "v_cndmask_b32 v20, v20, v16, vcc\n\t" \
         "v_cndmask_b32_e64 v20, v20, v14, s[48:49]\n\t" \
         "v_cndmask_b32_e64 v20, v20, v12, s[50:51]\n\t"
-#define NASTAR_ASM_SELECT \
-  \
-        "v_min_u32_dpp v22, v21, v21 quad_perm:[1,0,3,2] row_mask:0xf bank_mask:0xf\n\t" \
-        "s_nop 1\n\t" \
-        "v_min_u32_dpp v22, v22, v22 quad_perm:[2,3,0,1] row_mask:0xf bank_mask:0xf\n\t" \
-        "s_nop 1\n\t" \
-        "v_min_u32_dpp v22, v22, v22 row_half_mirror row_mask:0xf bank_mask:0xf\n\t" \
-        "s_nop 1\n\t" \
-        "v_min_u32_dpp v22, v22, v22 row_mirror row_mask:0xf bank_mask:0xf\n\t" \
+ \
+
+#define NASTAR_ASM_FIN_4 \
         "s_nop 1\n\t" \
         "v_min_u32_dpp v22, v22, v22 row_bcast:15 row_mask:0xa bank_mask:0xf\n\t" \
         "s_nop 1\n\t" \
         "v_min_u32_dpp v22, v22, v22 row_bcast:31 row_mask:0xc bank_mask:0xf\n\t" \
         "s_nop 0\n\t" \
-        "v_readlane_b32 s40, v22, 63\n\t"  \
+        "v_readlane_b32 s40, v22, 63\n\t"
+#define NASTAR_ASM_FIN_2 \
+        "s_nop 0\n\t" \
+        "v_readlane_b32 s40, v22, 0\n\t" \
+        "v_readlane_b32 s53, v22, 16\n\t" \
+        "s_min_u32 s40, s40, s53\n\t"
+#define NASTAR_ASM_FIN_1 \
+        "s_nop 0\n\t" \
+        "v_readlane_b32 s40, v22, 0\n\t"
+#define NASTAR_ASM_SELECT(FIN) \
+  \
+        "v_min_u32_dpp v22, v21, v21 quad_perm:[1,0,3,2] row_mask:0xf bank_mask:0xf\n\t" \
+        "s_nop 1\n\t" \
+        "v_min_u32_dpp v22, v22, v22 quad_perm:[2,3,0,1] row_mask:0xf bank_mask:0xf\n\t" \
+        "s_nop 1\n\t" \
+        "v_min_u32_dpp v22, v22, v22 row_half_mirror row_mask:0xf bank_mask:0xf\n\t" \
+        "s_nop 1\n\t" \
+        "v_min_u32_dpp v22, v22, v22 row_mirror row_mask:0xf bank_mask:0xf\n\t" \
+        FIN \
         "s_cmp_eq_u32 s40, -1\n\t" \
         "s_cbranch_scc1 .Lempty%=\n\t"  \
         "v_cmp_eq_u32 vcc, s40, v21\n\t" \
@@ -78,7 +92,7 @@
   \
         "s_lshr_b32 s43, s42, %[LOGW]\n\t"  \
         "s_and_b32 s44, s42, %[WM1]\n\t"  \
-        "s_and_b32 s45, s42, 0xfffffff0\n\t"  \
+        "s_and_b32 s45, s42, %[CBASE]\n\t"  \
         "v_add_u32 v23, s43, %[dr]\n\t" \
         "v_add_u32 v24, s44, %[dc]\n\t" \
         "v_max_u32 v23, v23, v24\n\t" \
@@ -109,10 +123,10 @@
         "v_sub_f32 v35, v35, v32\n\t"  \
         "v_mul_f32 v34, 0x3a83126f, v34\n\t"  \
         "v_add_f32 v34, v35, v34\n\t"  \
-        "s_lshr_b32 s47, s42, 4\n\t" \
+        "s_lshr_b32 s47, s42, %[CCL]\n\t" \
         "s_lshl_b32 s47, s47, 3\n\t"  \
-        "s_and_b32 s46, s42, 15\n\t" \
-        "s_add_u32 s46, s46, 16\n\t"  \
+        "s_and_b32 s46, s42, %[CCM1]\n\t" \
+        "s_add_u32 s46, s46, %[CLANE0]\n\t"  \
         "s_waitcnt lgkmcnt(0)\n\t" \
         "v_add_f32 v34, v34, v31\n\t"  \
         "v_mul_f32 v34, %[comg], v34\n\t"  \
@@ -128,7 +142,7 @@
         "v_bitop3_b32 v47, v43, v42, %[msb] bitop3:0x36\n\t"  \
         "v_cndmask_b32_e64 v45, %[vinf], v40, s[54:55]\n\t"  \
         "v_cndmask_b32 v44, %[loc], %[vinf], vcc\n\t"  \
-        "v_lshrrev_b32 v50, 4, v46\n\t" \
+        "v_lshrrev_b32 v50, %[CCL], v46\n\t" \
         "v_lshlrev_b32 v50, 3, v50\n\t"  \
         "v_mov_b32 v52, s47\n\t" \
   \
@@ -159,12 +173,13 @@
         "s_mov_b32 %[sel], s42\n" \
         ".Lend%=:\n\t"
 #define NASTAR_ASM_OPERANDS \
-        : [it] "+s"(it), [sel] "=s"(sel) \
+        : [it] "+&s"(it), [sel] "=s"(sel) \
         : [l8] "v"(v_l8), [lane] "v"(lane), [dr] "v"(v_dr), [dc] "v"(v_dc), [off] "v"(v_off), [pcode] "v"(v_pcode), \
           [vinf] "v"(v_inf), [vminf] "v"(v_minf), [loc] "v"(v_loc), [goal] "s"(goal_idx), [gr] "s"(goal_r), [gc] "s"(goal_c), \
           [maxit] "s"(max_iters), [cgr] "s"(d.gr), [comg] "s"(d.omg), [csq] "s"(d.sqrtW), [crcp] "s"(rcp_sqrtW), \
           [mnb] "s"(m_nb), [mchk] "s"(m_chk), [msb] "s"(msb), [logp] "s"(logp), \
-          [GC] "i"(L::GC), [CMIN] "i"(L::CMIN), [CMIN16] "i"(L::CMIN + 16), [PDIR] "i"(L::PDIR), [LOGW] "i"(LOGW), [WM1] "i"(L::W - 1), [W] "i"(L::W) \
+          [GC] "i"(L::GC), [CMIN] "i"(L::CMIN), [CMIN16] "i"(L::CMIN + 16), [PDIR] "i"(L::PDIR), [LOGW] "i"(LOGW), [WM1] "i"(L::W - 1), [W] "i"(L::W), \
+          [CCL] "i"(L::CCL), [CCM1] "i"((1 << L::CCL) - 1), [CBASE] "i"(~((1u << L::CCL) - 1u)), [CLANE0] "i"(L::ROWS == 2 ? 32 : 16) \
         : "memory", "vcc", "scc", "v20", "v21", "v22", "v23", "v24", "v26", "v27", "v28", "v29", "v30", "v31", "v32", "v33", \
           "v34", "v35", "v40", "v41", "v42", "v43", "v44", "v45", "v46", "v47", "v48", "v49", "v50", "v52", "s40", "s41", "s42", \
           "s43", "s44", "s45", "s46", "s47", "s50", "s51", "s52", "s54", "s55", "s53", "v53", "v54", "v12", "v13", "v14", "v15", "v16", "v17", "v18", "v19", "s48", "s49"
@@ -174,17 +189,17 @@
                                                        int max_iters, int& iters, float rcp_sqrtW, int* log_row)
 {
     using L = AsmLayout<LOGW>;
-    static_assert((L::CPL == 1 || L::CPL == 4) && L::HW >= 256, "1 or 4 chunk minima per lane, chunks inside one map row");
+    static_assert((L::CPL == 1 || L::CPL == 4) && L::HW >= 256 && (1 << L::CCL) <= L::W, "1 or 4 chunk minima per lane, chunks inside one map row");
     int dr, dc;
     neighbour_delta(lane & 7, dr, dc);
-    const bool is_nb = lane < 8, is_chk = (lane & 48) == 16;
+    const bool is_nb = lane < 8, is_chk = L::ROWS == 2 ? lane >= 32 : (lane & 48) == 16;
     const int v_dr = is_nb ? dr : 0, v_dc = is_nb ? dc : 0;
-    const int v_off = is_nb ? dr * L::W + dc : (is_chk ? (lane & 15) : 0);
+    const int v_off = is_nb ? dr * L::W + dc : (is_chk ? (lane & ((1 << L::CCL) - 1)) : 0);
     const uint32_t v_pcode = P_PASS | (uint32_t)(lane & 7);
     const uint32_t v_l8 = (uint32_t)lane * 8u * L::CPL;
     const float v_inf = NASTAR_POS_INF, v_minf = NASTAR_NEG_INF;
     const float v_loc = is_chk ? NASTAR_NEG_INF : NASTAR_POS_INF;
-    const unsigned long long m_nb = 0xFFull, m_chk = 0xFFFF0000ull;
+    const unsigned long long m_nb = 0xFFull, m_chk = L::ROWS == 2 ? 0xFFFFFFFF00000000ull : 0xFFFF0000ull;
     const uint32_t msb = 0x80000000u;
     int it = __builtin_amdgcn_readfirstlane(iters);
     goal_idx = __builtin_amdgcn_readfirstlane(goal_idx);
@@ -193,16 +208,19 @@
     max_iters = __builtin_amdgcn_readfirstlane(max_iters);
     int sel;
     unsigned long long logp = reinterpret_cast<unsigned long long>(log_row);
-#define NASTAR_ASM_BODY(N, LOGPART) \
-    NASTAR_ASM_ENTRY NASTAR_ASM_READ_##N NASTAR_ASM_LOOPTOP NASTAR_ASM_LOCALMIN_##N NASTAR_ASM_SELECT LOGPART NASTAR_ASM_EXPAND \
+#define NASTAR_ASM_BODY(N, FIN, LOGPART) \
+    NASTAR_ASM_ENTRY NASTAR_ASM_READ_##N NASTAR_ASM_LOOPTOP NASTAR_ASM_LOCALMIN_##N NASTAR_ASM_SELECT(FIN) LOGPART NASTAR_ASM_EXPAND \
         NASTAR_ASM_READ_##N NASTAR_ASM_LOOPEND
-    if constexpr (L::CPL == 1) {
-        if constexpr (kLog) asm volatile(NASTAR_ASM_BODY(1, NASTAR_ASM_LOG) NASTAR_ASM_OPERANDS);
-        else asm volatile(NASTAR_ASM_BODY(1, ) NASTAR_ASM_OPERANDS);
-    } else {
-        if constexpr (kLog) asm volatile(NASTAR_ASM_BODY(4, NASTAR_ASM_LOG) NASTAR_ASM_OPERANDS);
-        else asm volatile(NASTAR_ASM_BODY(4, ) NASTAR_ASM_OPERANDS);
-    }
+#define NASTAR_ASM_RUN(N, FIN) \
+    do { \
+        if constexpr (kLog) asm volatile(NASTAR_ASM_BODY(N, FIN, NASTAR_ASM_LOG) NASTAR_ASM_OPERANDS); \
+        else asm volatile(NASTAR_ASM_BODY(N, FIN, ) NASTAR_ASM_OPERANDS); \
+    } while (0)
+    if constexpr (L::CPL == 4) NASTAR_ASM_RUN(4, NASTAR_ASM_FIN_4);
+    else if constexpr (L::ROWS == 4) NASTAR_ASM_RUN(1, NASTAR_ASM_FIN_4);
+    else if constexpr (L::ROWS == 2) NASTAR_ASM_RUN(1, NASTAR_ASM_FIN_2);
+    else NASTAR_ASM_RUN(1, NASTAR_ASM_FIN_1);
+#undef NASTAR_ASM_RUN
 #undef NASTAR_ASM_BODY
     iters = it;
     return sel;
diff --git a/neural-astar_amd/csrc/nastar_search_asm3.hip.h b/neural-astar_amd/csrc/nastar_search_asm3.hip.h
--- a/neural-astar_amd/csrc/nastar_search_asm3.hip.h
+++ b/neural-astar_amd/csrc/nastar_search_asm3.hip.h
@@ -3,7 +3,7 @@
 
 namespace nastar {
 
-#define NASTAR_ASM3_SELECT \
+#define NASTAR_ASM3_SELECT(FIN) \
   \
         "v_min_u32_dpp v22, v21, v21 quad_perm:[1,0,3,2] row_mask:0xf bank_mask:0xf\n\t" \
         "v_min_u32_dpp v23, v21, v21 quad_perm:[2,3,0,1] row_mask:0xf bank_mask:0xf\n\t" \
@@ -14,12 +14,7 @@
         "v_min_u32_dpp v22, v22, v22 row_half_mirror row_mask:0xf bank_mask:0xf\n\t" \
         "s_nop 1\n\t" \
         "v_min_u32_dpp v22, v22, v22 row_mirror row_mask:0xf bank_mask:0xf\n\t" \
-        "s_nop 1\n\t" \
-        "v_min_u32_dpp v22, v22, v22 row_bcast:15 row_mask:0xa bank_mask:0xf\n\t" \
-        "s_nop 1\n\t" \
-        "v_min_u32_dpp v22, v22, v22 row_bcast:31 row_mask:0xc bank_mask:0xf\n\t" \
-        "s_nop 0\n\t" \
-        "v_readlane_b32 s40, v22, 63\n\t"  \
+        FIN  \
         "s_cmp_eq_u32 s40, -1\n\t" \
         "s_cbranch_scc1 .Lempty%=\n\t"  \
         "v_cmp_eq_u32 vcc, s40, v21\n\t" \
@@ -66,7 +61,7 @@
         "s_and_b64 s[54:55], vcc, %[mnb]\n\t"  \
         "v_cndmask_b32 v46, v24, v46, vcc\n\t"  \
         "v_lshlrev_b32 v26, 3, v46\n\t" \
-        "v_lshrrev_b32 v50, 4, v46\n\t" \
+        "v_lshrrev_b32 v50, %[CCL], v46\n\t" \
         "v_lshlrev_b32 v50, 3, v50\n\t"
 #define NASTAR_ASM3_X_CLOSE \
   \
@@ -159,12 +154,12 @@
 
 
 #define NASTAR_ASM3_OPERANDS \
-        : [it] "+s"(it), [sel] "=s"(sel) \
+        : [it] "+&s"(it), [sel] "=s"(sel) \
         : [l8] "v"(v_l8), [dr] "v"(v_dr), [cmask] "v"(v_cmask), [dcc] "v"(v_dcc), [pcode] "v"(v_pcode), [cls] "v"(v_cls), \
           [vminf] "v"(v_minf), [goal] "s"(goal_idx), [gr] "s"(goal_r), [gc] "s"(goal_c), \
           [maxit] "s"(max_iters), [cgr] "s"(d.gr), [comg] "s"(d.omg), [csq] "s"(d.sqrtW), [crcp] "s"(rcp_sqrtW), \
           [mnb] "s"(m_nb), [logp] "s"(logp), \
-          [GC] "i"(L::GC), [CMIN] "i"(L::CMIN), [CMIN16] "i"(L::CMIN + 16), [PDIR] "i"(L::PDIR), [LOGW] "i"(LOGW), [WM1] "i"(L::W - 1), [W] "i"(L::W) \
+          [GC] "i"(L::GC), [CMIN] "i"(L::CMIN), [CMIN16] "i"(L::CMIN + 16), [PDIR] "i"(L::PDIR), [LOGW] "i"(LOGW), [WM1] "i"(L::W - 1), [W] "i"(L::W), [CCL] "i"(L::CCL) \
         : "memory", "vcc", "scc", "v20", "v21", "v22", "v23", "v24", "v26", "v27", "v28", "v29", "v30", "v31", "v32", "v33", \
           "v34", "v35", "v36", "v37", "v40", "v41", "v42", "v43", "v46", "v47", "v48", "v49", "v50", "s40", "s41", "s42", \
           "s43", "s44", "s54", "s55", "s53", "v53", "v54", "v12", "v13", "v14", "v15", "v16", "v17", "v18", "v19", "s48", "s49", \
@@ -175,13 +170,13 @@
                                                         int max_iters, int& iters, float rcp_sqrtW, int* log_row)
 {
     using L = AsmLayout<LOGW>;
-    static_assert((L::CPL == 1 || L::CPL == 4) && L::HW >= 256, "1 or 4 chunk minima per lane, chunks inside one map row");
+    static_assert((L::CPL == 1 || L::CPL == 4) && L::HW >= 256 && (1 << L::CCL) <= L::W, "1 or 4 chunk minima per lane, chunks inside one map row");
     int dr, dc;
     neighbour_delta(lane & 7, dr, dc);
-    const bool is_nb = lane < 8, is_chk = (lane & 48) == 16;
+    const bool is_nb = lane < 8, is_chk = L::ROWS == 2 ? lane >= 32 : (lane & 48) == 16;
     const int v_dr = is_nb ? dr : 0;
-    const int v_dcc = is_nb ? dc : (is_chk ? (lane & 15) : 0);
-    const uint32_t v_cmask = is_chk ? 0xFFFFFFF0u : 0xFFFFFFFFu;
+    const int v_dcc = is_nb ? dc : (is_chk ? (lane & ((1 << L::CCL) - 1)) : 0);
+    const uint32_t v_cmask = is_chk ? ~((1u << L::CCL) - 1u) : 0xFFFFFFFFu;
     const uint32_t v_cls = is_chk ? 0x1F8u : 0u;
     const uint32_t v_pcode = P_PASS | (uint32_t)(lane & 7);
     const uint32_t v_l8 = (uint32_t)lane * 8u * L::CPL;
@@ -194,23 +189,25 @@
     max_iters = __builtin_amdgcn_readfirstlane(max_iters);
     int sel;
     unsigned long long logp = reinterpret_cast<unsigned long long>(log_row);
-#define NASTAR_ASM3_BODY(N, LOGPART) \
-    NASTAR_ASM_ENTRY NASTAR_ASM_READ_##N NASTAR_ASM_LOOPTOP NASTAR_ASM_LOCALMIN_##N NASTAR_ASM3_SELECT LOGPART NASTAR_ASM3_EXPAND \
+#define NASTAR_ASM3_BODY(N, FIN, LOGPART) \
+    NASTAR_ASM_ENTRY NASTAR_ASM_READ_##N NASTAR_ASM_LOOPTOP NASTAR_ASM_LOCALMIN_##N NASTAR_ASM3_SELECT(FIN) LOGPART NASTAR_ASM3_EXPAND \
         NASTAR_ASM_READ_##N NASTAR_ASM3_LOOPEND
-#define NASTAR_ASM3_BODY_DIVE(N, LOGPART) \
+#define NASTAR_ASM3_BODY_DIVE(N, FIN, LOGPART) \
     NASTAR_ASM_ENTRY NASTAR_ASM_READ_##N "s_branch .Lsel%=\n" NASTAR_ASM3_DIVE_LOOKUP LOGPART NASTAR_ASM3_EXPAND_DIVE NASTAR_ASM_READ_##N \
-        NASTAR_ASM3_DIVE_TEST ".Lsel%=:\n\t" "s_waitcnt lgkmcnt(0)\n\t" NASTAR_ASM_LOCALMIN_##N NASTAR_ASM3_SELECT \
+        NASTAR_ASM3_DIVE_TEST ".Lsel%=:\n\t" "s_waitcnt lgkmcnt(0)\n\t" NASTAR_ASM_LOCALMIN_##N NASTAR_ASM3_SELECT(FIN) \
         "s_branch .Lselected%=\n" NASTAR_ASM3_EXITS
+#define NASTAR_ASM3_RUN(BODY, N, FIN) \
+    do { \
+        if constexpr (kLog) asm volatile(BODY(N, FIN, NASTAR_ASM3_LOG) NASTAR_ASM3_OPERANDS); \
+        else asm volatile(BODY(N, FIN, ) NASTAR_ASM3_OPERANDS); \
+    } while (0)
     if constexpr (L::CPL == 1) {
-        if constexpr (kLog) asm volatile(NASTAR_ASM3_BODY(1, NASTAR_ASM3_LOG) NASTAR_ASM3_OPERANDS);
-        else asm volatile(NASTAR_ASM3_BODY(1, ) NASTAR_ASM3_OPERANDS);
-    } else if constexpr (kDive) {
-        if constexpr (kLog) asm volatile(NASTAR_ASM3_BODY_DIVE(4, NASTAR_ASM3_LOG) NASTAR_ASM3_OPERANDS);
-        else asm volatile(NASTAR_ASM3_BODY_DIVE(4, ) NASTAR_ASM3_OPERANDS);
-    } else {
-        if constexpr (kLog) asm volatile(NASTAR_ASM3_BODY(4, NASTAR_ASM3_LOG) NASTAR_ASM3_OPERANDS);
-        else asm volatile(NASTAR_ASM3_BODY(4, ) NASTAR_ASM3_OPERANDS);
-    }
+        if constexpr (L::ROWS == 4) NASTAR_ASM3_RUN(NASTAR_ASM3_BODY, 1, NASTAR_ASM_FIN_4);
+        else if constexpr (L::ROWS == 2) NASTAR_ASM3_RUN(NASTAR_ASM3_BODY, 1, NASTAR_ASM_FIN_2);
+        else NASTAR_ASM3_RUN(NASTAR_ASM3_BODY, 1, NASTAR_ASM_FIN_1);
+    } else if constexpr (kDive) NASTAR_ASM3_RUN(NASTAR_ASM3_BODY_DIVE, 4, NASTAR_ASM_FIN_4);
+    else NASTAR_ASM3_RUN(NASTAR_ASM3_BODY, 4, NASTAR_ASM_FIN_4);
+#undef NASTAR_ASM3_RUN
 #undef NASTAR_ASM3_BODY_DIVE
 #undef NASTAR_ASM3_BODY
     iters = it;
diff --git a/neural-astar_amd/csrc/nastar_search_asm4.hip.h b/neural-astar_amd/csrc/nastar_search_asm4.hip.h
--- a/neural-astar_amd/csrc/nastar_search_asm4.hip.h
+++ b/neural-astar_amd/csrc/nastar_search_asm4.hip.h
@@ -20,7 +20,27 @@
         "v_mov_b32 v48, %[goal]\n\t"  \
         "v_mov_b32 v49, -1\n\t"
 
-#define NASTAR_ASM4_SELECT \
+ \
+
+#define NASTAR_ASM4_FIN_4 \
+        "s_nop 1\n\t" \
+        "v_min_u32_dpp v22, v22, v22 row_bcast:15 row_mask:0xa bank_mask:0xf\n\t" \
+        "s_nop 1\n\t" \
+        "v_min_u32_dpp v22, v22, v22 row_bcast:31 row_mask:0xc bank_mask:0xf\n\t" \
+        "s_nop 0\n\t" \
+        "v_readlane_b32 s40, v22, 63\n\t"  \
+        "s_add_u32 %[it], %[it], 1\n\t"  \
+        "s_nop 0\n\t"
+#define NASTAR_ASM4_FIN_2 \
+        "s_add_u32 %[it], %[it], 1\n\t"  \
+        "v_readlane_b32 s40, v22, 0\n\t"  \
+        "v_readlane_b32 s53, v22, 16\n\t"  \
+        "s_min_u32 s40, s40, s53\n\t"
+#define NASTAR_ASM4_FIN_1 \
+        "s_add_u32 %[it], %[it], 1\n\t"  \
+        "v_readlane_b32 s40, v22, 0\n\t" \
+        "s_nop 1\n\t"
+#define NASTAR_ASM4_SELECT(FIN) \
         "v_min_u32_dpp v22, v21, v21 quad_perm:[1,0,3,2] row_mask:0xf bank_mask:0xf\n\t" \
         "v_min_u32_dpp v23, v21, v21 quad_perm:[2,3,0,1] row_mask:0xf bank_mask:0xf\n\t" \
         "v_min_u32_dpp v22, v21, v22 quad_perm:[3,2,1,0] row_mask:0xf bank_mask:0xf\n\t" \
@@ -29,14 +49,7 @@
         "v_min_u32_dpp v22, v22, v22 row_half_mirror row_mask:0xf bank_mask:0xf\n\t" \
         "s_nop 1\n\t" \
         "v_min_u32_dpp v22, v22, v22 row_mirror row_mask:0xf bank_mask:0xf\n\t" \
-        "s_nop 1\n\t" \
-        "v_min_u32_dpp v22, v22, v22 row_bcast:15 row_mask:0xa bank_mask:0xf\n\t" \
-        "s_nop 1\n\t" \
-        "v_min_u32_dpp v22, v22, v22 row_bcast:31 row_mask:0xc bank_mask:0xf\n\t" \
-        "s_nop 0\n\t" \
-        "v_readlane_b32 s40, v22, 63\n\t"  \
-        "s_add_u32 %[it], %[it], 1\n\t"  \
-        "s_nop 0\n\t" \
+        FIN \
         "v_cmp_eq_u32 vcc, s40, v21\n\t" \
         "s_ff1_i32_b64 s41, vcc\n\t" \
         "v_readlane_b32 s42, v20, s41\n\t" \
@@ -57,7 +70,7 @@
         RDS  \
         "v_lshlrev_b32 v26, " SH ", v46\n\t" \
         "s_and_b64 s[54:55], vcc, %[mnb]\n\t"  \
-        "v_lshrrev_b32 v50, 4, v46\n\t" \
+        "v_lshrrev_b32 v50, %[CCL], v46\n\t" \
         "v_lshlrev_b32 v50, 3, v50\n\t"
 
 #define NASTAR_ASM4_X_KEY(ADDH, ADDG, MULH, MULG) \
@@ -109,12 +122,12 @@
         NASTAR_ASM4_EXITS
 
 #define NASTAR_ASM4_OPERANDS \
-        : [it] "+s"(it), [sel] "=s"(sel), [mkey] "=s"(mkey) \
+        : [it] "+&s"(it), [sel] "=s"(sel), [mkey] "=s"(mkey) \
         : [l8] "v"(v_l8), [dr] "v"(v_dr), [cmask] "v"(v_cmask), [dcc] "v"(v_dcc), [pcode] "v"(v_pcode), [cls] "v"(v_cls), \
           [vminf] "v"(v_minf), [goal] "s"(goal_idx), [gr] "s"(goal_r), [gc] "s"(goal_c), \
           [maxit] "s"(max_iters), [cgr] "s"(cgr), [comg] "s"(comg), [csq] "s"(csq), [crcp] "s"(rcp_sqrtW), \
           [mnb] "s"(m_nb), [logp] "s"(logp), \
-          [GC] "i"(GC), [CMIN] "i"(CMIN), [CMIN16] "i"(CMIN + 16), [PDIR] "i"(PDIR), [LOGW] "i"(LOGW), [WM1] "i"((1 << LOGW) - 1), [W] "i"(1 << LOGW) \
+          [GC] "i"(GC), [CMIN] "i"(CMIN), [CMIN16] "i"(CMIN + 16), [PDIR] "i"(PDIR), [LOGW] "i"(LOGW), [WM1] "i"((1 << LOGW) - 1), [W] "i"(1 << LOGW), [CCL] "i"(CCLS) \
         : "memory", "vcc", "scc", "v20", "v21", "v22", "v23", "v24", "v26", "v27", "v28", "v29", "v30", "v31", "v32", "v33", \
           "v34", "v35", "v36", "v37", "v40", "v41", "v42", "v43", "v46", "v47", "v48", "v49", "v50", "s40", "s41", "s42", \
           "s43", "s44", "s54", "s55", "s53", "v53", "v54", "v12", "v13", "v14", "v15", "v16", "v17", "v18", "v19", "s48", "s49", \
@@ -130,13 +143,15 @@
     constexpr int GC = kUnit ? LU::GC : LG::GC;
     constexpr int CMIN = kUnit ? LU::CMIN : LG::CMIN;
     constexpr int PDIR = kUnit ? LU::PDIR : LG::PDIR;
-    static_assert((CPL == 1 || CPL == 4) && LG::HW >= 256, "1 or 4 chunk minima per lane, chunks inside one map row");
+    constexpr int CCLS = kUnit ? CCL : LG::CCL;
+    constexpr int ROWS = CPL > 1 ? 4 : ((LG::HW >> CCLS) + 15) / 16;
+    static_assert((CPL == 1 || CPL == 4) && LG::HW >= 256 && (1 << CCLS) <= LG::W, "1 or 4 chunk minima per lane, chunks inside one map row");
     int dr, dc;
     neighbour_delta(lane & 7, dr, dc);
-    const bool is_nb = lane < 8, is_chk = (lane & 48) == 16;
+    const bool is_nb = lane < 8, is_chk = CCLS == 5 ? lane >= 32 : (lane & 48) == 16;
     const int v_dr = is_nb ? dr : 0;
-    const int v_dcc = is_nb ? dc : (is_chk ? (lane & 15) : 0);
-    const uint32_t v_cmask = is_chk ? 0xFFFFFFF0u : 0xFFFFFFFFu;
+    const int v_dcc = is_nb ? dc : (is_chk ? (lane & ((1 << CCLS) - 1)) : 0);
+    const uint32_t v_cmask = is_chk ? ~((1u << CCLS) - 1u) : 0xFFFFFFFFu;
     const uint32_t v_cls = is_chk ? 0x1F8u : 0u;
     const uint32_t v_pcode = P_PASS | (uint32_t)(lane & 7);
     const uint32_t v_l8 = (uint32_t)lane * 8u * CPL;
@@ -165,29 +180,35 @@
 #define NASTAR_A4_EXPAND(L, MH, MG, SET55) \
     NASTAR_ASM4_X_PREFIX(NASTAR_A4_SH_##L, NASTAR_A4_RDS_##L) NASTAR_ASM3_X_CLOSE NASTAR_A4_RDC_##L NASTAR_ASM3_X_HEUR NASTAR_ASM3_X_WAIT \
         NASTAR_ASM4_X_KEY(NASTAR_A4_ADDH_##L, NASTAR_A4_ADDG_##L, MH, MG) NASTAR_ASM3_X_RELAX(SET55)
-#define NASTAR_A4_BODY(N, L, MH, MG, LOGPART) \
-    NASTAR_ASM4_ENTRY NASTAR_ASM_READ_##N NASTAR_ASM_LOOPTOP NASTAR_ASM_LOCALMIN_##N NASTAR_ASM4_SELECT LOGPART NASTAR_A4_EXPAND(L, MH, MG, ) \
+#define NASTAR_A4_BODY(N, L, MH, MG, FIN, LOGPART) \
+    NASTAR_ASM4_ENTRY NASTAR_ASM_READ_##N NASTAR_ASM_LOOPTOP NASTAR_ASM_LOCALMIN_##N NASTAR_ASM4_SELECT(FIN) LOGPART NASTAR_A4_EXPAND(L, MH, MG, ) \
         NASTAR_ASM_READ_##N NASTAR_ASM4_LOOPEND
-#define NASTAR_A4_BODY_DIVE(N, L, MH, MG, LOGPART) \
+#define NASTAR_A4_BODY_DIVE(N, L, MH, MG, FIN, LOGPART) \
     NASTAR_ASM4_ENTRY NASTAR_ASM_READ_##N "s_branch .Lsel%=\n" NASTAR_ASM4_DIVE_LOOKUP LOGPART \
         NASTAR_A4_EXPAND(L, MH, MG, "v_cmp_lt_u32_e64 s[60:61], v47, s40\n\t") NASTAR_ASM_READ_##N NASTAR_ASM3_DIVE_TEST ".Lsel%=:\n\t" \
-        "s_waitcnt lgkmcnt(0)\n\t" NASTAR_ASM_LOCALMIN_##N NASTAR_ASM4_SELECT "s_branch .Lselected%=\n" NASTAR_ASM4_EXITS
-#define NASTAR_A4_RUN2(BODY, N, L, MH, MG) \
+        "s_waitcnt lgkmcnt(0)\n\t" NASTAR_ASM_LOCALMIN_##N NASTAR_ASM4_SELECT(FIN) "s_branch .Lselected%=\n" NASTAR_ASM4_EXITS
+#define NASTAR_A4_RUN2(BODY, N, L, MH, MG, FIN) \
     do { \
-        if constexpr (kLog) asm volatile(BODY(N, L, MH, MG, NASTAR_ASM3_LOG) NASTAR_ASM4_OPERANDS); \
-        else asm volatile(BODY(N, L, MH, MG, ) NASTAR_ASM4_OPERANDS); \
+        if constexpr (kLog) asm volatile(BODY(N, L, MH, MG, FIN, NASTAR_ASM3_LOG) NASTAR_ASM4_OPERANDS); \
+        else asm volatile(BODY(N, L, MH, MG, FIN, ) NASTAR_ASM4_OPERANDS); \
     } while (0)
-#define NASTAR_A4_RUN(BODY, N) \
+#define NASTAR_A4_RUN(BODY, N, FIN) \
     do { \
-        if constexpr (kUnit && kHalf) NASTAR_A4_RUN2(BODY, N, U, , ); \
-        else if constexpr (kUnit) NASTAR_A4_RUN2(BODY, N, U, NASTAR_A4_MULH, NASTAR_A4_MULG); \
-        else if constexpr (kHalf) NASTAR_A4_RUN2(BODY, N, G, , ); \
-        else NASTAR_A4_RUN2(BODY, N, G, NASTAR_A4_MULH, NASTAR_A4_MULG); \
+        if constexpr (kUnit && kHalf) NASTAR_A4_RUN2(BODY, N, U, , , FIN); \
+        else if constexpr (kUnit) NASTAR_A4_RUN2(BODY, N, U, NASTAR_A4_MULH, NASTAR_A4_MULG, FIN); \
+        else if constexpr (kHalf) NASTAR_A4_RUN2(BODY, N, G, , , FIN); \
+        else NASTAR_A4_RUN2(BODY, N, G, NASTAR_A4_MULH, NASTAR_A4_MULG, FIN); \
     } while (0)
-    if constexpr (CPL == 1 && kDive) NASTAR_A4_RUN(NASTAR_A4_BODY_DIVE, 1);
-    else if constexpr (CPL == 1) NASTAR_A4_RUN(NASTAR_A4_BODY, 1);
-    else if constexpr (kDive) NASTAR_A4_RUN(NASTAR_A4_BODY_DIVE, 4);
-    else NASTAR_A4_RUN(NASTAR_A4_BODY, 4);
+#define NASTAR_A4_RUN_ROWS(BODY) \
+    do { \
+        if constexpr (CPL == 4) NASTAR_A4_RUN(BODY, 4, NASTAR_ASM4_FIN_4); \
+        else if constexpr (ROWS == 4) NASTAR_A4_RUN(BODY, 1, NASTAR_ASM4_FIN_4); \
+        else if constexpr (ROWS == 2) NASTAR_A4_RUN(BODY, 1, NASTAR_ASM4_FIN_2); \
+        else NASTAR_A4_RUN(BODY, 1, NASTAR_ASM4_FIN_1); \
+    } while (0)
+    if constexpr (kDive) NASTAR_A4_RUN_ROWS(NASTAR_A4_BODY_DIVE);
+    else NASTAR_A4_RUN_ROWS(NASTAR_A4_BODY);
+#undef NASTAR_A4_RUN_ROWS
 #undef NASTAR_A4_RUN
 #undef NASTAR_A4_RUN2
 #undef NASTAR_A4_BODY_DIVE
diff --git a/neural-astar_amd/csrc/nastar_search_asm5.hip.h b/neural-astar_amd/csrc/nastar_search_asm5.hip.h
--- a/neural-astar_amd/csrc/nastar_search_asm5.hip.h
+++ b/neural-astar_amd/csrc/nastar_search_asm5.hip.h
@@ -21,7 +21,7 @@
 #define NASTAR_ASM5_X_SHADOW \
   \
         "v_readlane_b32 s54, %[colmask], s42\n\t" \
-        "v_lshrrev_b32 v50, 4, v46\n\t" \
+        "v_lshrrev_b32 v50, %[CCL], v46\n\t" \
         "v_lshlrev_b32 v50, 3, v50\n\t"  \
         "s_mov_b64 exec, 0x100\n\t" \
         "ds_write_b64 v50, v[48:49] offset:%[CMIN]\n\t" \
@@ -41,12 +41,12 @@
 #define NASTAR_ASM5_MULG "v_mul_f32 v41, %[cgr], v41\n\t"
 
 #define NASTAR_ASM5_OPERANDS \
-        : [it] "+s"(it), [sel] "=s"(sel), [mkey] "=s"(mkey) \
+        : [it] "+&s"(it), [sel] "=s"(sel), [mkey] "=s"(mkey) \
         : [l8] "v"(v_l8), [cmask] "v"(v_cmask), [colmask] "v"(v_colmask), [delta] "v"(v_delta), [pcode] "v"(v_pcode), \
           [cls] "v"(v_cls), [vminf] "v"(v_minf), [goal] "s"(goal_idx), \
           [maxit] "s"(max_iters), [cgr] "s"(cgr), [comg] "s"(comg), [csq] "s"(csq), [crcp] "s"(rcp_sqrtW), \
           [mnb] "s"(m_nb), [logp] "s"(logp), \
-          [GC] "i"(GC), [CMIN] "i"(CMIN), [CMIN16] "i"(CMIN + 16), [PDIR] "i"(PDIR) \
+          [GC] "i"(GC), [CMIN] "i"(CMIN), [CMIN16] "i"(CMIN + 16), [PDIR] "i"(PDIR), [CCL] "i"(LG::CCL) \
         : "memory", "vcc", "scc", "v20", "v21", "v22", "v23", "v26", "v27", "v28", "v30", "v31", \
           "v40", "v41", "v42", "v43", "v46", "v47", "v48", "v49", "v50", "s40", "s41", "s42", \
           "s54", "s55", "s53", "v53", "v54", "v12", "v13", "v14", "v15", "v16", "v17", "v18", "v19", "s48", "s49", \
@@ -61,12 +61,13 @@
     constexpr int GC = LG::GC;
     constexpr int CMIN = LG::CMIN;
     constexpr int PDIR = LG::PDIR;
-    static_assert((CPL == 1 || CPL == 4) && LG::HW >= 256, "1 or 4 chunk minima per lane, chunks inside one map row");
+    constexpr int ROWS = LG::ROWS;
+    static_assert((CPL == 1 || CPL == 4) && LG::HW >= 256 && (1 << LG::CCL) <= LG::W, "1 or 4 chunk minima per lane, chunks inside one map row");
     int dr, dc;
     neighbour_delta(lane & 7, dr, dc);
-    const bool is_nb = lane < 8, is_chk = (lane & 48) == 16;
-    const int v_delta = is_nb ? dr * (1 << LOGW) + dc : (is_chk ? (lane & 15) : 0);
-    const uint32_t v_cmask = is_chk ? 0xFFFFFFF0u : 0xFFFFFFFFu;
+    const bool is_nb = lane < 8, is_chk = ROWS == 2 ? lane >= 32 : (lane & 48) == 16;
+    const int v_delta = is_nb ? dr * (1 << LOGW) + dc : (is_chk ? (lane & ((1 << LG::CCL) - 1)) : 0);
+    const uint32_t v_cmask = is_chk ? ~((1u << LG::CCL) - 1u) : 0xFFFFFFFFu;
     const uint32_t v_cls = is_chk ? 0x1F8u : 0u;
     const uint32_t v_pcode = P_PASS | (uint32_t)(lane & 7);
     const uint32_t v_l8 = (uint32_t)lane * 8u * CPL;
@@ -83,27 +84,33 @@
 #define NASTAR_A5_EXPAND(MH, MG, SET55) \
     NASTAR_ASM5_X_PREFIX NASTAR_ASM5_X_CLOSE NASTAR_ASM5_X_READCELL NASTAR_ASM5_X_SHADOW NASTAR_ASM5_X_WAIT NASTAR_ASM5_X_KEY(MH, MG) \
         NASTAR_ASM3_X_RELAX(SET55)
-#define NASTAR_A5_BODY(N, MH, MG, LOGPART) \
-    NASTAR_ASM5_ENTRY NASTAR_ASM4_ENTRY NASTAR_ASM_READ_##N NASTAR_ASM_LOOPTOP NASTAR_ASM_LOCALMIN_##N NASTAR_ASM4_SELECT LOGPART NASTAR_A5_EXPAND(MH, MG, ) \
+#define NASTAR_A5_BODY(N, MH, MG, FIN, LOGPART) \
+    NASTAR_ASM5_ENTRY NASTAR_ASM4_ENTRY NASTAR_ASM_READ_##N NASTAR_ASM_LOOPTOP NASTAR_ASM_LOCALMIN_##N NASTAR_ASM4_SELECT(FIN) LOGPART NASTAR_A5_EXPAND(MH, MG, ) \
         NASTAR_ASM_READ_##N NASTAR_ASM4_LOOPEND
-#define NASTAR_A5_BODY_DIVE(N, MH, MG, LOGPART) \
+#define NASTAR_A5_BODY_DIVE(N, MH, MG, FIN, LOGPART) \
     NASTAR_ASM5_ENTRY NASTAR_ASM4_ENTRY NASTAR_ASM_READ_##N "s_branch .Lsel%=\n" NASTAR_ASM4_DIVE_LOOKUP LOGPART \
         NASTAR_A5_EXPAND(MH, MG, "v_cmp_lt_u32_e64 s[60:61], v47, s40\n\t") NASTAR_ASM_READ_##N NASTAR_ASM3_DIVE_TEST ".Lsel%=:\n\t" \
-        "s_waitcnt lgkmcnt(0)\n\t" NASTAR_ASM_LOCALMIN_##N NASTAR_ASM4_SELECT "s_branch .Lselected%=\n" NASTAR_ASM4_EXITS
-#define NASTAR_A5_RUN2(BODY, N, MH, MG) \
+        "s_waitcnt lgkmcnt(0)\n\t" NASTAR_ASM_LOCALMIN_##N NASTAR_ASM4_SELECT(FIN) "s_branch .Lselected%=\n" NASTAR_ASM4_EXITS
+#define NASTAR_A5_RUN2(BODY, N, MH, MG, FIN) \
     do { \
-        if constexpr (kLog) asm volatile(BODY(N, MH, MG, NASTAR_ASM3_LOG) NASTAR_ASM5_OPERANDS); \
-        else asm volatile(BODY(N, MH, MG, ) NASTAR_ASM5_OPERANDS); \
+        if constexpr (kLog) asm volatile(BODY(N, MH, MG, FIN, NASTAR_ASM3_LOG) NASTAR_ASM5_OPERANDS); \
+        else asm volatile(BODY(N, MH, MG, FIN, ) NASTAR_ASM5_OPERANDS); \
     } while (0)
-#define NASTAR_A5_RUN(BODY, N) \
+#define NASTAR_A5_RUN(BODY, N, FIN) \
     do { \
-        if constexpr (kHalf) NASTAR_A5_RUN2(BODY, N, , ); \
-        else NASTAR_A5_RUN2(BODY, N, NASTAR_ASM5_MULH, NASTAR_ASM5_MULG); \
+        if constexpr (kHalf) NASTAR_A5_RUN2(BODY, N, , , FIN); \
+        else NASTAR_A5_RUN2(BODY, N, NASTAR_ASM5_MULH, NASTAR_ASM5_MULG, FIN); \
     } while (0)
-    if constexpr (CPL == 1 && kDive) NASTAR_A5_RUN(NASTAR_A5_BODY_DIVE, 1);
-    else if constexpr (CPL == 1) NASTAR_A5_RUN(NASTAR_A5_BODY, 1);
-    else if constexpr (kDive) NASTAR_A5_RUN(NASTAR_A5_BODY_DIVE, 4);
-    else NASTAR_A5_RUN(NASTAR_A5_BODY, 4);
+#define NASTAR_A5_RUN_ROWS(BODY) \
+    do { \
+        if constexpr (CPL == 4) NASTAR_A5_RUN(BODY, 4, NASTAR_ASM4_FIN_4); \
+        else if constexpr (ROWS == 4) NASTAR_A5_RUN(BODY, 1, NASTAR_ASM4_FIN_4); \
+        else if constexpr (ROWS == 2) NASTAR_A5_RUN(BODY, 1, NASTAR_ASM4_FIN_2); \
+        else NASTAR_A5_RUN(BODY, 1, NASTAR_ASM4_FIN_1); \
+    } while (0)
+    if constexpr (kDive) NASTAR_A5_RUN_ROWS(NASTAR_A5_BODY_DIVE);
+    else NASTAR_A5_RUN_ROWS(NASTAR_A5_BODY);
+#undef NASTAR_A5_RUN_ROWS
 #undef NASTAR_A5_RUN
 #undef NASTAR_A5_RUN2
 #undef NASTAR_A5_BODY_DIVE
diff --git a/neural-astar_amd/csrc/nastar_search_compact.hip.h b/neural-astar_amd/csrc/nastar_search_compact.hip.h
--- a/neural-astar_amd/csrc/nastar_search_compact.hip.h
+++ b/neural-astar_amd/csrc/nastar_search_compact.hip.h
@@ -5,6 +5,7 @@
 
 constexpr int CCL = 4;
 constexpr int CCSZ = 1 << CCL;
+__host__ __device__ constexpr int compact_asm_ccl(int logw) { return logw == 5 ? 5 : CCL; }
 
 struct CompactDims {
     int H, W, HW;
@@ -213,7 +214,7 @@
 
 template <bool kFastDiv>
 __device__ __forceinline__ void compact_open_start(const CompactDims& d, const CompactLds& l, int lane, int sidx, int goal_r,
-                                                   int goal_c, float rcp_sqrtW, bool raw_key = false, bool half_key = false)
+                                                   int goal_c, float rcp_sqrtW, bool raw_key = false, bool half_key = false, int ccl = CCL)
 {
     if (lane == 0) {
         const int r = (int)row_magic((uint32_t)sidx, d.magicW, d.W);
@@ -222,7 +223,7 @@
         uint32_t k0 = compact_key<kFastDiv>(d, 0.0f, hh, rcp_sqrtW);
         if (raw_key) k0 = __float_as_uint(ord_to_f32(k0));
         l.gc[sidx].x = 0.0f;
-        l.cmin[sidx >> CCL] = cmin_entry(k0, (uint32_t)sidx);
+        l.cmin[sidx >> ccl] = cmin_entry(k0, (uint32_t)sidx);
         l.pdir[sidx] = (uint8_t)(PARENT_UNSET | P_PASS);
     }
     wave_sync();
```

Measured after the change: 38.70 million (median of 6 runs). 2.8% higher.
